# icbi-lab/infercnvpy

Measured on AMD Instinct MI355X. Metric: cells/sec through tl.infercnv (window=100), input resident in HBM, higher is better.
Workload: dtype f64

## Files before the change

include/infercnv_hip.h:

```cpp
#ifndef INFERCNV_HIP_H
#define INFERCNV_HIP_H

#include <stdint.h>

#ifdef __cplusplus
extern "C" {
#endif

typedef enum {
    ICV_OK = 0,
    ICV_ERR_INVALID = 1,
    ICV_ERR_UNSUPPORTED = 2,
    ICV_ERR_HIP = 3,
    ICV_ERR_NOMEM = 4
} icv_status;

enum { ICV_F32 = 0, ICV_F64 = 1 };
enum { ICV_DENSE = 0, ICV_CSR = 1 };

enum {
    ICV_FLAG_TRUNC_TO_INT = 1,
    ICV_FLAG_ROUND_F32 = 2,
    ICV_FLAG_NO_APPLY = 4
};
// ... 8 lines not shown
    const void *values;
    const int64_t *indptr;
    const int32_t *indices;
    int64_t csr_begin;
    int64_t csr_end;
} icv_matrix;

typedef struct icv_plan_s *icv_plan_t;

typedef struct {
    int32_t n_cols_all;
    int32_t n_genes_used;
    int32_t n_chr;
    int32_t window;
    int32_t step;
    int32_t n_windows;
    int32_t block;
    int32_t n_blocks;
    int32_t padded_len;
    int32_t lds_bytes_f32;
    int32_t lds_bytes_f64;
    int32_t workgroups_per_cu_f32;
} icv_plan_info;

int icv_plan_create(int32_t n_cols_all, const int32_t *h_col_pos, int32_t n_chr,
                    const int32_t *h_chrom_offsets, int32_t window, int32_t step, icv_plan_t *out);
void icv_plan_destroy(icv_plan_t plan);
int icv_plan_get_info(icv_plan_t plan, icv_plan_info *h_info);
int icv_plan_chr_pos(icv_plan_t plan, int32_t *h_chr_pos );
int icv_plan_window_table(icv_plan_t plan, int32_t *h_start , int32_t *h_len );
enum {
    ICV_KERNEL_NONE = 0,
    ICV_KERNEL_GENERIC = 1,
    ICV_KERNEL_WS = 2,
    ICV_KERNEL_WS_CSR = 3,
    ICV_KERNEL_X16 = 4,
    ICV_KERNEL_SD = 5,
    ICV_KERNEL_SPLIT = 6
};
int icv_plan_last_kernel(icv_plan_t plan, int32_t *h_kind);
int icv_plan_se_tables(icv_plan_t plan, int32_t *h_applies, int32_t *h_col_block ,
                       int32_t *h_col_offset , int32_t *h_block_gene0 ,
                       uint32_t *h_w0 , uint32_t *h_w1 );
int icv_plan_gene_runs(icv_plan_t plan, int32_t *h_n_runs, int32_t *h_run_first, int32_t *h_run_count,
                       int32_t *h_run_genes, int32_t *h_col_run );

int icv_colsum(const icv_matrix *m, const int32_t *row_group, int32_t n_groups, double *sums,
               void *stream);

int icv_colchain(const icv_matrix *m, const int32_t *rows, int64_t n_sel, double scale, void *acc, void *stream);
int icv_colsum_pairwise(const void *xt, int32_t dtype, int64_t n_rows, int32_t n_cols, int64_t ld, void *sums,
                        void *stream);
int icv_colchain_mean(const void *acc, int32_t dtype, int32_t n_cols, int64_t count, void *mean, void *stream);
int icv_colmean_csc(const void *values, int32_t dtype, const int64_t *colptr, const int32_t *row_idx, int32_t n_cols,
                    const int32_t *row_group, int32_t group, double scale, void *mean, void *stream);

int icv_infercnv_smooth(icv_plan_t plan, const icv_matrix *m, const void *ref_lo, const void *ref_hi,
                        double lfc_clip, int32_t flags, float *out, int64_t ldo, double *cell_median,
                        double *cell_stats, void *stream);

int icv_chunk_thresholds(const double *cell_stats, int64_t n_rows, int64_t chunksize, int64_t row_phase,
                         int32_t n_windows, double dynamic_threshold, double *thr, void *stream);

int icv_apply_threshold(icv_plan_t plan, const icv_matrix *m, const void *ref_lo, const void *ref_hi,
                        double lfc_clip, int32_t flags, float *out, int64_t ldo,
                        const double *cell_median, const double *thr, int64_t chunksize,
                        int64_t row_phase, void *stream);

typedef struct {
    float smooth_ms;
    float thresholds_ms;
    float apply_ms;
    float total_ms;
} icv_profile;

int icv_infercnv_run(icv_plan_t plan, const icv_matrix *m, const void *ref_lo, const void *ref_hi,
                     double lfc_clip, double dynamic_threshold, int64_t chunksize, int64_t row_phase,
                     int32_t flags, float *out, int64_t ldo, double *cell_median, double *cell_stats,
                     double *thr, icv_profile *h_profile, void *stream);

int icv_profile_begin(icv_plan_t plan);
int icv_profile_collect(icv_plan_t plan, icv_profile *out, int32_t max_records, int32_t *n_records);

int icv_colchain_blocks_workspace(int64_t n_rows, int32_t n_cols, int64_t *bytes);
int icv_colchain_blocks_sums(const icv_matrix *m, void *workspace, double *total, void *stream);
int icv_colchain_blocks_records(const icv_matrix *m, void *workspace, const double *est_start, void *stream);
int icv_colchain_blocks_scan(const icv_matrix *m, void *workspace, float *acc, int32_t col0, int32_t col1,
                             uint64_t *d_replayed, void *stream);

int icv_infercnv_run_windows(icv_plan_t plan, const icv_matrix *m, const void *ref_lo, const void *ref_hi,
                             double lfc_clip, double dynamic_threshold, int64_t chunksize, int64_t row_phase,
                             int32_t flags, float *out, int64_t ldo, double *cell_median, double *cell_stats,
                             double *thr, icv_profile *h_profile, double *win_out, int64_t ldw, void *stream);
int icv_gene_values_from_windows(icv_plan_t plan, const double *win, int64_t ldw, int64_t n_rows,
                                 const double *thr, int64_t chunksize, int64_t row_phase, double *gene_out,
                                 int64_t ldg, void *stream);
int icv_gene_values(icv_plan_t plan, const icv_matrix *m, const void *ref_lo, const void *ref_hi,
                    double lfc_clip, int32_t flags, const double *thr, int64_t chunksize,
                    int64_t row_phase, double *gene_out, int64_t ldg, void *stream);

int icv_csr_count(const float *x, int64_t n_rows, int32_t n_cols, int64_t ld, int64_t *row_nnz, void *stream);
int icv_csr_fill(const float *x, int64_t n_rows, int32_t n_cols, int64_t ld, const int64_t *indptr,
                 int32_t *indices, double *data, void *stream);

typedef struct {
    int32_t rows_per_round;
    int32_t mask_streamed;
    int32_t mask_ring_slots;
    int32_t mask_lds_bytes;
    int32_t mask_loads_in_flight;
    int32_t fill_streamed;
    int32_t fill_ring_slots;
    int32_t fill_lds_bytes;
    int32_t fill_loads_in_flight;
    int32_t fill_stage_entries;
} icv_pack_info;
int icv_pack_geometry(int32_t n_windows, icv_pack_info *h_info);

int icv_threshold_mask(icv_plan_t plan, const icv_matrix *m, const void *ref_lo, const void *ref_hi,
                       double lfc_clip, int32_t flags, const float *out, int64_t ldo, const double *cell_median,
                       const double *thr, int64_t chunksize, int64_t row_phase, uint64_t *mask,
                       int64_t *row_nnz, void *stream);
int icv_csr_fill_masked(const float *x, int64_t n_rows, int32_t n_cols, int64_t ld, const uint64_t *mask,
                        const int64_t *indptr, int32_t *indices, double *data, void *stream);
int icv_row_offsets(const int64_t *row_nnz, int64_t n_rows, int64_t *indptr, void *stream);

int icv_threshold_pack(icv_plan_t plan, const icv_matrix *m, const void *ref_lo, const void *ref_hi, double lfc_clip,
                       int32_t flags, const float *out, int64_t ldo, const double *cell_median, const double *thr,
                       int64_t chunksize, int64_t row_phase, int64_t *indptr, int32_t *indices, double *data,
                       int64_t capacity, void *stream);

int icv_corr_iqr(const float *x, int64_t n, int32_t k, int64_t ld, double *h_iqr, void *stream);

int icv_pairwise_sqeuclidean(const float *x, int64_t n, int32_t d, int64_t ld, int64_t row_begin, int64_t row_end,
                             float *out, int64_t ldo, void *stream);
int icv_ward_linkage(float *dist_sq, int64_t n, int64_t ld, int32_t spare_columns, double *h_linkage,
                     int32_t *h_rounds, void *stream);

#define ICV_SUPER_ROWS 1024
int icv_pairwise_sqeuclidean_tiles(const float *x, int64_t n, int32_t d, int64_t ld, int32_t n_tiles,
                                   const int32_t *h_row0, const int32_t *h_col0, const int64_t *h_dir_off,
                                   const int64_t *h_mir_off, float *dir, int64_t ld_dir, float *mir, int64_t ld_mir,
                                   void *stream);

typedef struct icv_ward_s *icv_ward_t;
int icv_ward_create(int64_t n, const int32_t *h_sr_local, int32_t n_super, int32_t super_shift, int64_t ld,
                    int32_t spare_columns, icv_ward_t *out, void *stream);
void icv_ward_destroy(icv_ward_t w);
int icv_ward_merge(icv_ward_t w, float *d_local, int64_t ld, const float *stage, int64_t ld_stage,
                   const int32_t *h_pslot, int32_t scatter, void *stream);
int icv_ward_gather(icv_ward_t w, const float *d_local, int64_t ld, const int64_t *d_rows, int32_t n_rows,
                    const int32_t *d_slots, int32_t n_slots, float *out, int64_t ldo, void *stream);
int icv_ward_scatter(icv_ward_t w, float *d_local, int64_t ld, const float *v, int64_t ldv, const int32_t *h_vrow_p,
                     int32_t n_v, void *stream);
int icv_ward_scan(icv_ward_t w, const float *d_local, int64_t ld, void *stream);
int icv_ward_pack_nn(icv_ward_t w, int32_t *d_nn, float *d_dmin, void *stream);
int icv_ward_unpack_nn(icv_ward_t w, const int32_t *d_nn, const float *d_dmin, void *stream);
int icv_ward_pairs(icv_ward_t w, float *d_local, int64_t ld, int32_t all_active, int32_t *h_counts ,
                   void *stream);
int icv_ward_round_pairs(icv_ward_t w, int32_t *h_i, int32_t *h_j);
int icv_ward_finish(icv_ward_t w, double *h_linkage, int32_t *h_rounds);

int icv_row_abs_sum(const float *x, int64_t n_rows, int32_t n_cols, int64_t ld, double *row_sum,
                    void *stream);

int icv_csr_row_abs_sum(const void *data, int32_t dtype, const int64_t *indptr, int64_t n_rows, double *row_sum,
                        void *stream);

int icv_group_sums(const double *values, const int32_t *group, int64_t n, int32_t n_groups, double *sums,
                   int64_t *counts, void *stream);

int icv_csr_check(const int64_t *indptr, const int32_t *indices, int64_t n_rows, int32_t n_cols, int64_t capacity,
                  void *stream);
int icv_csr_densify(const void *data, int32_t dtype, const int64_t *indptr, const int32_t *indices, const int64_t *rows,
                    int64_t n_sel, int32_t n_cols, float *out, int64_t ldo, void *stream);

#define ICV_GRAM_BLOCK 8192
int icv_gram_f64(const icv_matrix *m, int32_t panel_dtype, void *panel, int64_t panel_ld, double *g, int64_t ldg,
// ... 47 lines not shown
```

infercnvpy_amd/_engine.py:

```python
from __future__ import annotations

import ctypes as C
import math
import os
import time as _time

import numpy as np
import scipy.sparse as sp

from . import _lib
from ._plan import GenePlan


def _torch():
    import torch

    if not torch.cuda.is_available():
        raise RuntimeError("infercnvpy_amd needs an AMD GPU (torch.cuda.is_available() is False); "
                           "there is no CPU fallback")
    return torch


def _stream_ptr(torch):
    return C.c_void_p(torch.cuda.current_stream().cuda_stream)
# ... 161 lines not shown
        if not count:
            raise ValueError("column_chain: CSR input needs the row count of the group")
        scale = 1.0 / float(count)
    _lib.check(lib.icv_colchain(C.byref(m), _ptr(rows_d), n_sel, scale, C.c_void_p(acc_ptr), _stream_ptr(torch)))
    return acc


class ChainBlocks:

    def __init__(self, dm: "DeviceMatrix", row0=0, row1=None):
        torch = _torch()
        lib = _lib.load()
        self.dm = dm
        self.m = dm.c_struct(row0, row1)
        nbytes = C.c_int64(0)
        _lib.check(lib.icv_colchain_blocks_workspace(self.m.n_rows, self.m.n_cols, C.byref(nbytes)))
        self.ws = torch.empty(int(nbytes.value), dtype=torch.uint8, device="cuda")
        self.replayed = torch.zeros(1, dtype=torch.int64, device="cuda")

    def sums(self):
        torch = _torch()
        total = torch.empty(self.m.n_cols, dtype=torch.float64, device="cuda")
        _lib.check(_lib.load().icv_colchain_blocks_sums(C.byref(self.m), _ptr(self.ws), _ptr(total), _stream_ptr(torch)))
        return total

    def records(self, est_start=None):
        torch = _torch()
        if est_start is not None:
            assert est_start.dtype == torch.float64 and est_start.is_cuda and est_start.numel() == self.m.n_cols
            est_start = est_start.contiguous()
        _lib.check(_lib.load().icv_colchain_blocks_records(C.byref(self.m), _ptr(self.ws), _ptr(est_start),
                                                           _stream_ptr(torch)))

    def scan(self, acc, cols=None):
        torch = _torch()
        assert acc.dtype == torch.float32 and acc.is_cuda and acc.numel() == self.m.n_cols and acc.is_contiguous()
        c0, c1 = (0, self.m.n_cols) if cols is None else (int(cols[0]), int(cols[1]))
        _lib.check(_lib.load().icv_colchain_blocks_scan(C.byref(self.m), _ptr(self.ws), _ptr(acc), c0, c1,
                                                        _ptr(self.replayed), _stream_ptr(torch)))
        return acc

    def n_blocks(self):
        return (-(-int(self.m.n_rows) // 64)) * int(self.m.n_cols)


def chain_mean(acc, count, is_csr):
    if is_csr:
        return acc
    torch = _torch()
    lib = _lib.load()
    out = torch.empty_like(acc)
    _lib.check(lib.icv_colchain_mean(_ptr(acc), _lib.ICV_F32 if acc.dtype == torch.float32 else _lib.ICV_F64,
                                     acc.numel(), int(count), _ptr(out), _stream_ptr(torch)))
    return out


def csc_column_means(X, row_group=None, n_groups=1, counts=None, np_dtype=None, max_entries=1 << 28):
    torch = _torch()
    lib = _lib.load()
    X = X.tocsc()
    if not X.has_canonical_format:
        X = X.copy()
        X.sum_duplicates()
    np_dtype = np.dtype(np_dtype or (np.float32 if X.dtype == np.float32 else np.float64))
    tdt = torch.float32 if np_dtype == np.float32 else torch.float64
    code = _lib.ICV_F32 if np_dtype == np.float32 else _lib.ICV_F64
    n_cols = X.shape[1]
    indptr = X.indptr.astype(np.int64, copy=False)
    out = np.zeros((n_groups, n_cols), dtype=np_dtype)
    rg = None
    if row_group is not None:
        rg = torch.from_numpy(np.ascontiguousarray(row_group, dtype=np.int32)).cuda()
    if counts is None:
        counts = [X.shape[0]] * n_groups
    c = 0
    while c < n_cols:
        c1 = int(np.searchsorted(indptr, indptr[c] + max_entries, side="right")) - 1
        c1 = min(n_cols, max(c1, c + 1))
        e0, e1 = int(indptr[c]), int(indptr[c1])
        vals = torch.from_numpy(np.ascontiguousarray(X.data[e0:e1].astype(np_dtype, copy=False))).cuda()
        rows = torch.from_numpy(np.ascontiguousarray(X.indices[e0:e1].astype(np.int32, copy=False))).cuda()
        ptr = torch.from_numpy(np.ascontiguousarray(indptr[c:c1 + 1] - e0)).cuda()
        if e1 == e0:
            vals = torch.zeros(1, dtype=tdt, device="cuda")
            rows = torch.zeros(1, dtype=torch.int32, device="cuda")
        for g in range(n_groups):
            mean = torch.empty(c1 - c, dtype=tdt, device="cuda")
            _lib.check(lib.icv_colmean_csc(_ptr(vals), code, _ptr(ptr), _ptr(rows), c1 - c, _ptr(rg), g,
                                           1.0 / float(counts[g]), _ptr(mean), _stream_ptr(torch)))
            out[g, c:c1] = mean.cpu().numpy()
        c = c1
    return out


def fortran_column_means(X, np_dtype=None, max_bytes=1 << 30):
    torch = _torch()
    lib = _lib.load()
    n, g = X.shape
    np_dtype = np.dtype(np_dtype or (np.float32 if X.dtype == np.float32 else np.float64))
    tdt = torch.float32 if np_dtype == np.float32 else torch.float64
    code = _lib.ICV_F32 if np_dtype == np.float32 else _lib.ICV_F64
    XT = X.T
    out = np.empty(g, dtype=np_dtype)
    per = int(max(1, max_bytes // max(1, n * np_dtype.itemsize)))
    for c0 in range(0, g, per):
        c1 = min(g, c0 + per)
# ... 294 lines not shown
            th.start()

    @property
    def h2d_seconds(self):
        return max(self._busy)

    def pieces(self):
        torch = _torch()
        for k in range(len(self.bounds)):
            if k >= self._landed:
                for q in self._queues:
                    ev = q.get()
                    if ev is None:
                        raise self._err
                    torch.cuda.current_stream().wait_event(ev)
                self._landed += 1
            yield self.bounds[k]
        self._join()

    def _join(self):
        for th in self._threads:
            if th.is_alive():
                th.join()

    def close(self, cancel=False):
        if cancel:
            self._cancel.set()
        self._join()
        bufs_q = getattr(self, "_pack_bufs", None)
        if bufs_q is not None:
            self._pack_bufs = None
            while True:
                try:
                    _pack_pool_give(bufs_q.get_nowait())
                except Exception:
                    break
        if self.dm is not None:
            torch = _torch()
            cur = torch.cuda.current_stream()
            for t in self.dm._keep:
                t.record_stream(cur)
                for st in self._streams:
                    t.record_stream(st)
        self.dm = None


class PackedRows:

    def __init__(self, out, mask, counts, thr):
        self.out, self.mask, self.counts, self.thr = out, mask, counts, thr


def threshold_mask(plan: GenePlan, dm: DeviceMatrix, ref_lo, ref_hi, res, *, lfc_clip, chunksize, row_phase=0,
                   flags=0, row0=0, row1=None):
    torch = _torch()
    lib = _lib.load()
    rows = res.out.shape[0]
    n_words = (plan.n_windows + 63) // 64
    mask = torch.empty((rows, n_words), dtype=torch.int64, device="cuda")
    counts = torch.empty(rows, dtype=torch.int64, device="cuda")
    m = dm.c_struct(row0, row1)
    _lib.check(lib.icv_threshold_mask(
        plan.handle, C.byref(m), _ptr(ref_lo), _ptr(ref_hi), float(lfc_clip), int(flags), _ptr(res.out),
        res.out.stride(0), _ptr(res.cell_median), _ptr(res.thr), int(chunksize), int(row_phase), _ptr(mask),
        _ptr(counts), _stream_ptr(torch)))
    return PackedRows(res.out, mask, counts, res.thr)


class PackedCsr:

    def __init__(self, indptr, indices, data, n_cols, thr=None):
        self.indptr, self.indices, self.data, self.n_cols, self.thr = indptr, indices, data, n_cols, thr

    @property
    def n_rows(self):
        return self.indptr.shape[0] - 1

    @property
    def shape(self):
        return (self.n_rows, self.n_cols)

    @property
    def device(self):
        return self.indptr.device

    def nnz(self):
        return int(self.indptr[-1].item())

    def to_scipy(self):
        ip = self.indptr.cpu().numpy()
        n = int(ip[-1])
        return sp.csr_matrix((self.data[:n].cpu().numpy(), self.indices[:n].cpu().numpy(), ip),
                             shape=(self.n_rows, self.n_cols))

    def toarray(self):
        return self.to_scipy().toarray()

    def dense_rows(self, rows=None):
        torch = _torch()
        lib = _lib.load()
        with torch.cuda.device(self.device):
            rows_d, n_sel = None, self.n_rows
            if rows is not None:
                rows = np.asarray(rows)
                if rows.dtype == bool:
                    if rows.shape[0] != self.n_rows:
                        raise IndexError("boolean row mask of the wrong length")
                    rows = np.flatnonzero(rows)
                rows = np.ascontiguousarray(rows, dtype=np.int64)
                if rows.size and (rows.min() < 0 or rows.max() >= self.n_rows):
                    raise IndexError("row index out of range")
                n_sel = int(rows.shape[0])
                rows_d = torch.from_numpy(rows).cuda()
            ld = (self.n_cols + 3) // 4 * 4
            out = torch.empty((n_sel, max(ld, 1)), dtype=torch.float32, device="cuda")[:, :self.n_cols]
            code = _lib.ICV_F32 if self.data.dtype == torch.float32 else _lib.ICV_F64
            _lib.check(lib.icv_csr_densify(_ptr(self.data), code, _ptr(self.indptr), _ptr(self.indices), _ptr(rows_d),
                                           n_sel, self.n_cols, _ptr(out), out.stride(0), _stream_ptr(torch)))
        return out


def threshold_csr(plan: GenePlan, dm: DeviceMatrix, ref_lo, ref_hi, res, *, lfc_clip, chunksize, row_phase=0,
                  flags=0, row0=0, row1=None, capacity=None, single_pass=False):
    torch = _torch()
    lib = _lib.load()
    rows = res.out.shape[0]
    W = plan.n_windows
    if (dm.shape[0] if row1 is None else row1) - row0 == 0:
        return PackedCsr(torch.zeros(1, dtype=torch.int64, device="cuda"), torch.empty(1, dtype=torch.int32, device="cuda"),
                         torch.empty(1, dtype=torch.float64, device="cuda"), W, res.thr)
    if single_pass and W <= 20480:
        return threshold_pack(plan, dm, ref_lo, ref_hi, res, lfc_clip=lfc_clip, chunksize=chunksize,
                              row_phase=row_phase, flags=flags, row0=row0, row1=row1, capacity=capacity)
    part = threshold_mask(plan, dm, ref_lo, ref_hi, res, lfc_clip=lfc_clip, chunksize=chunksize, row_phase=row_phase,
                          flags=flags, row0=row0, row1=row1)
    cap = rows * W if capacity is None else max(int(capacity), rows * W)
    indptr = torch.empty(rows + 1, dtype=torch.int64, device="cuda")
    indices = torch.empty(max(cap, 1), dtype=torch.int32, device="cuda")
    data = torch.empty(max(cap, 1), dtype=torch.float64, device="cuda")
    st = _stream_ptr(torch)
    _lib.check(lib.icv_row_offsets(_ptr(part.counts), rows, _ptr(indptr), st))
    if rows:
        _lib.check(lib.icv_csr_fill_masked(_ptr(part.out), rows, W, part.out.stride(0), _ptr(part.mask), _ptr(indptr),
                                           _ptr(indices), _ptr(data), st))
    return PackedCsr(indptr, indices, data, W, res.thr)


def threshold_pack(plan: GenePlan, dm: DeviceMatrix, ref_lo, ref_hi, res, *, lfc_clip, chunksize, row_phase=0,
                   flags=0, row0=0, row1=None, capacity=None):
    torch = _torch()
    lib = _lib.load()
    rows = res.out.shape[0]
    W = plan.n_windows
    cap = rows * W if capacity is None else int(capacity)
    indptr = torch.empty(rows + 1, dtype=torch.int64, device="cuda")
    indices = torch.empty(max(cap, 1), dtype=torch.int32, device="cuda")
    data = torch.empty(max(cap, 1), dtype=torch.float64, device="cuda")
    m = dm.c_struct(row0, row1)
    _lib.check(lib.icv_threshold_pack(
        plan.handle, C.byref(m), _ptr(ref_lo), _ptr(ref_hi), float(lfc_clip), int(flags), _ptr(res.out),
        res.out.stride(0), _ptr(res.cell_median), _ptr(res.thr), int(chunksize), int(row_phase), _ptr(indptr),
        _ptr(indices), _ptr(data), cap, _stream_ptr(torch)))
    return PackedCsr(indptr, indices, data, W, res.thr)


def fill_from_mask(part, n_cols):
    torch = _torch()
    lib = _lib.load()
    n = part.counts.shape[0]
    ip = torch.zeros(n + 1, dtype=torch.int64, device="cuda")
    torch.cumsum(part.counts, 0, out=ip[1:])
    nnz = int(ip[-1].item())
    idx = torch.empty(max(nnz, 1), dtype=torch.int32, device="cuda")
    dat = torch.empty(max(nnz, 1), dtype=torch.float64, device="cuda")
    if nnz:
        _lib.check(lib.icv_csr_fill_masked(_ptr(part.out), n, n_cols, part.out.stride(0), _ptr(part.mask), _ptr(ip),
                                           _ptr(idx), _ptr(dat), _stream_ptr(torch)))
    return PackedCsr(ip, idx, dat, n_cols, part.thr)


def concat_packed(parts):
    torch = _torch()
    ips, idx, dat, thr, off = [parts[0].indptr[:1]], [], [], [], 0
    for p in parts:
        n = p.nnz()
        ips.append(p.indptr[1:] + off)
        idx.append(p.indices[:n])
        dat.append(p.data[:n])
        if p.thr is not None:
            thr.append(p.thr)
        off += n
    return PackedCsr(torch.cat(ips), torch.cat(idx), torch.cat(dat), parts[0].n_cols, torch.cat(thr) if thr else None)


# ... 692 lines not shown
```

infercnvpy_amd/_lib.py:

```python
from __future__ import annotations

import ctypes as C
import os

_HERE = os.path.dirname(os.path.abspath(__file__))
LIB_PATH = os.environ.get("INFERCNV_HIP_LIB") or os.path.join(_HERE, "libinfercnv_hip.so")

ICV_OK, ICV_ERR_INVALID, ICV_ERR_UNSUPPORTED, ICV_ERR_HIP, ICV_ERR_NOMEM = range(5)
ICV_F32, ICV_F64 = 0, 1
ICV_DENSE, ICV_CSR = 0, 1
ICV_FLAG_TRUNC_TO_INT = 1
ICV_FLAG_ROUND_F32 = 2
ICV_FLAG_NO_APPLY = 4
ICV_GRAM_BLOCK = 8192
(ICV_KERNEL_NONE, ICV_KERNEL_GENERIC, ICV_KERNEL_WS, ICV_KERNEL_WS_CSR, ICV_KERNEL_X16, ICV_KERNEL_SD,
 ICV_KERNEL_SPLIT) = range(7)

EXPORTS = (
    "icv_plan_create", "icv_plan_destroy", "icv_plan_get_info", "icv_plan_chr_pos", "icv_plan_window_table",
    "icv_plan_last_kernel", "icv_plan_se_tables", "icv_plan_gene_runs",
    "icv_colsum", "icv_colchain", "icv_colsum_pairwise", "icv_colchain_mean", "icv_colmean_csc", "icv_infercnv_smooth", "icv_chunk_thresholds", "icv_apply_threshold", "icv_infercnv_run",
    "icv_infercnv_run_windows", "icv_gene_values_from_windows",
    "icv_colchain_blocks_workspace", "icv_colchain_blocks_sums", "icv_colchain_blocks_records", "icv_colchain_blocks_scan",
    "icv_profile_begin", "icv_profile_collect",
    "icv_gene_values", "icv_csr_count", "icv_csr_fill", "icv_threshold_mask", "icv_csr_fill_masked", "icv_row_offsets", "icv_pack_geometry", "icv_threshold_pack", "icv_corr_iqr",
    "icv_pairwise_sqeuclidean", "icv_ward_linkage", "icv_pairwise_sqeuclidean_tiles",
    "icv_ward_create", "icv_ward_destroy", "icv_ward_merge", "icv_ward_gather", "icv_ward_scatter", "icv_ward_scan", "icv_ward_pack_nn",
    "icv_ward_unpack_nn", "icv_ward_pairs", "icv_ward_round_pairs", "icv_ward_finish", "icv_row_abs_sum", "icv_csr_row_abs_sum", "icv_group_sums", "icv_csr_check", "icv_csr_densify", "icv_gram_f64", "icv_project", "icv_host_dense_row_nnz", "icv_host_dense_pack", "icv_host_dense_pack_fused", "icv_csr_scatter_dense", "icv_last_error", "icv_version",
    "icv_device_count", "icv_developer_knobs_reload",
    "icv_knn_workspace", "icv_knn", "icv_knn_fuzzy", "icv_knn_symmetrize_count", "icv_knn_symmetrize_fill",
    "icv_knn_sort_rows",
    "icv_leiden_workspace", "icv_leiden_quantise", "icv_leiden_iteration", "icv_leiden_sums", "icv_leiden_renumber",
)


class Matrix(C.Structure):
    _fields_ = [
        ("format", C.c_int32), ("dtype", C.c_int32), ("n_rows", C.c_int64), ("n_cols", C.c_int32),
        ("_pad", C.c_int32), ("ld", C.c_int64), ("values", C.c_void_p), ("indptr", C.c_void_p),
        ("indices", C.c_void_p), ("csr_begin", C.c_int64), ("csr_end", C.c_int64),
    ]


class PlanInfo(C.Structure):
    _fields_ = [(n, C.c_int32) for n in (
        "n_cols_all", "n_genes_used", "n_chr", "window", "step", "n_windows", "block", "n_blocks", "padded_len",
        "lds_bytes_f32", "lds_bytes_f64", "workgroups_per_cu_f32")]


class PackInfo(C.Structure):
    _fields_ = [(n, C.c_int32) for n in (
        "rows_per_round", "mask_streamed", "mask_ring_slots", "mask_lds_bytes", "mask_loads_in_flight", "fill_streamed",
        "fill_ring_slots", "fill_lds_bytes", "fill_loads_in_flight", "fill_stage_entries")]


class Profile(C.Structure):
    _fields_ = [("smooth_ms", C.c_float), ("thresholds_ms", C.c_float), ("apply_ms", C.c_float),
                ("total_ms", C.c_float)]


class HipExtensionMissing(RuntimeError):
    pass


_lib = None


def load():
    global _lib
    if _lib is not None:
        return _lib
    if not os.path.exists(LIB_PATH):
        raise HipExtensionMissing(
            f"{LIB_PATH} not found: build it with `python -m infercnvpy_amd._build` "
            "(hipcc --offload-arch=gfx950).  infercnvpy_amd has no CPU fallback."
        )
    import torch

    lib = C.CDLL(LIB_PATH)
    i32, i64, vp, dbl = C.c_int32, C.c_int64, C.c_void_p, C.c_double
    P = C.POINTER
    lib.icv_plan_create.argtypes = [i32, vp, i32, vp, i32, i32, P(vp)]
    lib.icv_plan_destroy.argtypes = [vp]
    lib.icv_plan_destroy.restype = None
    lib.icv_plan_get_info.argtypes = [vp, P(PlanInfo)]
    lib.icv_plan_chr_pos.argtypes = [vp, vp]
    lib.icv_plan_window_table.argtypes = [vp, vp, vp]
    lib.icv_plan_last_kernel.argtypes = [vp, P(i32)]
    lib.icv_plan_se_tables.argtypes = [vp, P(i32), vp, vp, vp, vp, vp]
    lib.icv_plan_gene_runs.argtypes = [vp, P(i32), vp, vp, vp, vp]
    lib.icv_colsum.argtypes = [P(Matrix), vp, i32, vp, vp]
    lib.icv_colchain.argtypes = [P(Matrix), vp, i64, dbl, vp, vp]
    lib.icv_colsum_pairwise.argtypes = [vp, i32, i64, i32, i64, vp, vp]
    lib.icv_colchain_mean.argtypes = [vp, i32, i32, i64, vp, vp]
    lib.icv_colmean_csc.argtypes = [vp, i32, vp, vp, i32, vp, i32, dbl, vp, vp]
    lib.icv_infercnv_smooth.argtypes = [vp, P(Matrix), vp, vp, dbl, i32, vp, i64, vp, vp, vp]
    lib.icv_chunk_thresholds.argtypes = [vp, i64, i64, i64, i32, dbl, vp, vp]
    lib.icv_apply_threshold.argtypes = [vp, P(Matrix), vp, vp, dbl, i32, vp, i64, vp, vp, i64, i64, vp]
    lib.icv_infercnv_run.argtypes = [vp, P(Matrix), vp, vp, dbl, dbl, i64, i64, i32, vp, i64, vp, vp, vp,
                                     P(Profile), vp]
    lib.icv_infercnv_run_windows.argtypes = [vp, P(Matrix), vp, vp, dbl, dbl, i64, i64, i32, vp, i64, vp, vp, vp,
                                             P(Profile), vp, i64, vp]
    lib.icv_gene_values_from_windows.argtypes = [vp, vp, i64, i64, vp, i64, i64, vp, i64, vp]
    lib.icv_colchain_blocks_workspace.argtypes = [i64, i32, P(i64)]
    lib.icv_colchain_blocks_sums.argtypes = [P(Matrix), vp, vp, vp]
    lib.icv_colchain_blocks_records.argtypes = [P(Matrix), vp, vp, vp]
    lib.icv_colchain_blocks_scan.argtypes = [P(Matrix), vp, vp, i32, i32, vp, vp]
    lib.icv_profile_begin.argtypes = [vp]
    lib.icv_profile_collect.argtypes = [vp, P(Profile), i32, P(i32)]
    lib.icv_gene_values.argtypes = [vp, P(Matrix), vp, vp, dbl, i32, vp, i64, i64, vp, i64, vp]
    lib.icv_csr_count.argtypes = [vp, i64, i32, i64, vp, vp]
    lib.icv_csr_fill.argtypes = [vp, i64, i32, i64, vp, vp, vp, vp]
    lib.icv_threshold_mask.argtypes = [vp, P(Matrix), vp, vp, dbl, i32, vp, i64, vp, vp, i64, i64, vp, vp, vp]
    lib.icv_threshold_pack.argtypes = [vp, P(Matrix), vp, vp, dbl, i32, vp, i64, vp, vp, i64, i64, vp, vp, vp, i64, vp]
    lib.icv_row_offsets.argtypes = [vp, i64, vp, vp]
    lib.icv_pack_geometry.argtypes = [i32, P(PackInfo)]
    lib.icv_csr_fill_masked.argtypes = [vp, i64, i32, i64, vp, vp, vp, vp, vp]
    lib.icv_corr_iqr.argtypes = [vp, i64, i32, i64, P(C.c_double), vp]
    lib.icv_pairwise_sqeuclidean.argtypes = [vp, i64, i32, i64, i64, i64, vp, i64, vp]
    lib.icv_ward_linkage.argtypes = [vp, i64, i64, i32, vp, P(i32), vp]
    lib.icv_pairwise_sqeuclidean_tiles.argtypes = [vp, i64, i32, i64, i32, vp, vp, vp, vp, vp, i64, vp, i64, vp]
    lib.icv_ward_create.argtypes = [i64, vp, i32, i32, i64, i32, P(vp), vp]
    lib.icv_ward_destroy.argtypes = [vp]
    lib.icv_ward_destroy.restype = None
    lib.icv_ward_merge.argtypes = [vp, vp, i64, vp, i64, vp, i32, vp]
    lib.icv_ward_gather.argtypes = [vp, vp, i64, vp, i32, vp, i32, vp, i64, vp]
    lib.icv_ward_scatter.argtypes = [vp, vp, i64, vp, i64, vp, i32, vp]
    lib.icv_ward_scan.argtypes = [vp, vp, i64, vp]
    lib.icv_ward_pack_nn.argtypes = [vp, vp, vp, vp]
    lib.icv_ward_unpack_nn.argtypes = [vp, vp, vp, vp]
    lib.icv_ward_pairs.argtypes = [vp, vp, i64, i32, P(i32), vp]
    lib.icv_ward_round_pairs.argtypes = [vp, vp, vp]
    lib.icv_ward_finish.argtypes = [vp, vp, P(i32)]
    lib.icv_row_abs_sum.argtypes = [vp, i64, i32, i64, vp, vp]
    lib.icv_csr_row_abs_sum.argtypes = [vp, i32, vp, i64, vp, vp]
    lib.icv_group_sums.argtypes = [vp, vp, i64, i32, vp, vp, vp]
    lib.icv_csr_check.argtypes = [vp, vp, i64, i32, i64, vp]
    lib.icv_csr_densify.argtypes = [vp, i32, vp, vp, vp, i64, i32, vp, i64, vp]
    lib.icv_gram_f64.argtypes = [P(Matrix), i32, vp, i64, vp, i64, i32, vp]
    lib.icv_project.argtypes = [P(Matrix), vp, i32, vp, i32, vp, i64, vp]
    lib.icv_host_dense_row_nnz.argtypes = [vp, i32, i64, i64, i64, vp, i32]
    lib.icv_host_dense_pack.argtypes = [vp, i32, i64, i64, i64, vp, vp, vp, i32]
    lib.icv_host_dense_pack_fused.argtypes = [vp, i32, i64, i64, i64, vp, vp, vp, i64, i32, vp]
    lib.icv_csr_scatter_dense.argtypes = [vp, i32, vp, vp, i64, i32, vp, i64, vp]
    lib.icv_knn_workspace.argtypes = [i64, i32, i32, P(i64)]
    lib.icv_knn.argtypes = [vp, i64, i32, i64, i32, vp, vp, vp, P(i32), P(C.c_float), vp]
    lib.icv_knn_fuzzy.argtypes = [vp, i64, i32, vp, vp, vp, vp]
    lib.icv_knn_symmetrize_count.argtypes = [vp, vp, i64, i32, vp, vp]
    lib.icv_knn_symmetrize_fill.argtypes = [vp, vp, i64, i32, vp, i64, vp, vp, vp]
    lib.icv_knn_sort_rows.argtypes = [vp, i64, vp, vp, vp, vp, vp]
    lib.icv_leiden_workspace.argtypes = [i64, i64, P(i64)]
    lib.icv_leiden_quantise.argtypes = [vp, vp, vp, i32, i64, i64, i32, vp, vp, vp, P(i64), vp]
    lib.icv_leiden_iteration.argtypes = [vp, vp, vp, i64, i64, dbl, C.c_uint64, i32, vp, vp, P(i32), P(i32), P(i64),
                                         P(i32), P(C.c_float), vp]
    lib.icv_leiden_sums.argtypes = [vp, vp, vp, i64, vp, vp, vp, vp]
    lib.icv_leiden_renumber.argtypes = [vp, i64, vp, P(i32), vp]
    lib.icv_developer_knobs_reload.restype = None
    lib.icv_developer_knobs_reload.argtypes = []
    lib.icv_last_error.restype = C.c_char_p
    lib.icv_last_error.argtypes = []
    for name in EXPORTS:
        fn = getattr(lib, name)
        if name not in ("icv_plan_destroy", "icv_ward_destroy", "icv_last_error", "icv_developer_knobs_reload"):
            fn.restype = C.c_int
    _lib = lib
    return lib


# ... 16 lines not shown
```

infercnvpy_amd/csrc/icv_api.hip:

```cpp
#include "../../include/infercnv_hip.h"

#include <hip/hip_runtime.h>

#include <algorithm>
#include <atomic>
#include <cmath>
#include <cstdio>
#include <cstdlib>
#include <cstring>
#include <mutex>
#include <new>
#include <string>
#include <system_error>
#include <thread>
#if defined(__x86_64__)
#include <immintrin.h>
#endif
#include <memory>
#include <vector>

#include <rocprim/device/device_radix_sort.hpp>
#include <rocprim/device/device_reduce_by_key.hpp>
#include <rocprim/device/device_scan.hpp>

// ... 44 lines not shown
        no_x16 = std::getenv("ICV_NO_X16") != nullptr;
        no_sd = std::getenv("ICV_NO_SD") != nullptr;
        phase_profile = std::getenv("ICV_PHASE_PROFILE") != nullptr;
        ward_in_place = std::getenv("ICV_WARD_IN_PLACE") != nullptr;
        no_mask_ring = std::getenv("ICV_NO_MASK_RING") != nullptr;
        no_fill_ring = std::getenv("ICV_NO_FILL_RING") != nullptr;
        no_chain_queues = std::getenv("ICV_NO_CHAIN_QUEUES") != nullptr;
        se_maxw4 = std::getenv("ICV_SE_MAXW4") != nullptr;
        no_gene_fused = std::getenv("ICV_NO_GENE_FUSED") != nullptr;
        const char* e = std::getenv("ICV_WGS_PER_CU");
        wgs_per_cu = e ? std::atoi(e) : 0;
        e = std::getenv("ICV_CHAIN_FAR");
        chain_far = e ? std::atoi(e) : 0;
        e = std::getenv("ICV_CHAIN_PIECES");
        chain_pieces = e ? std::atoi(e) : 0;
        e = std::getenv("ICV_WARD_COMPACT_X");
        ward_compact_x = e ? std::atof(e) : 0.0;
    }
};
std::mutex g_knobs_mu;
bool g_knobs_loaded = false;
Knobs g_knobs;
const Knobs& knobs() {
    std::lock_guard<std::mutex> lk(g_knobs_mu);
    if (!g_knobs_loaded) {
        g_knobs.load();
        g_knobs_loaded = true;
    }
    return g_knobs;
}

}

struct icv_plan_s {
    icv::Plan p;
    std::mutex mu;
    std::atomic<bool> busy{false};
    int device = -1;
    int n_cu = 0;
    int32_t *d_dst = nullptr, *d_src = nullptr, *d_wstart = nullptr, *d_wlen = nullptr;
    double* d_wdenom = nullptr;
    int32_t* d_pad = nullptr;
    int32_t* d_wpack = nullptr;
    unsigned* d_tie_n = nullptr;
    int32_t *d_cov_col = nullptr, *d_cov_j0 = nullptr, *d_cov_cnt = nullptr;
    uint32_t* d_gv_pk = nullptr;
    int32_t* d_gv_mult = nullptr;
    uint16_t* d_gv_col16 = nullptr;
    bool gv_fused_ok = false;
    int gv_mult_bytes = 2;
    int64_t* d_row_list = nullptr;
    int* d_row_count = nullptr;
    int64_t row_list_cap = 0;
    bool prof_deferred = false;
    std::vector<hipEvent_t> prof_events;
    double* d_win_scratch = nullptr;
    int64_t win_scratch_cap = 0;
    double* d_cell_part = nullptr;
    int64_t cell_part_cap = 0;
    double* d_chunk_part = nullptr;
    int64_t chunk_part_cap = 0;
    double* d_hb_stats = nullptr;
    int64_t hb_stats_cap = 0;
    uint16_t* d_dst16 = nullptr;
    uint32_t* d_x16_wdesc = nullptr;
    int32_t* d_blk_g0 = nullptr;
    uint32_t *d_se_w0 = nullptr, *d_se_w1 = nullptr;
    void* d_zrow = nullptr;
    size_t zrow_elems = 0;
    std::vector<icv_plan_s*> parts;
    std::vector<int> part_woff;
    int parts_elem = 0;
    int last_kernel = ICV_KERNEL_NONE;
    hipEvent_t done_ev = nullptr;
    hipStream_t last_stream = nullptr;
    bool has_last = false;
};

namespace {

int64_t se_grid(const icv_plan_t pl, int64_t n_rows) {
    int per_cu = icv::kLdsLimit / icv::kSeLds;
    if (const int v = knobs().wgs_per_cu)
        if (v >= 1 && v < per_cu) per_cu = v;
    int64_t grid = (int64_t)pl->n_cu * per_cu;
    return grid > n_rows ? n_rows : grid;
}

struct PlanBusy {
    icv_plan_t pl;
    bool ok;
    hipStream_t st = nullptr;
    bool entered = false;
    explicit PlanBusy(icv_plan_t p) : pl(p), ok(false) {
        bool expected = false;
        ok = p && p->busy.compare_exchange_strong(expected, true);
    }
    hipError_t enter(hipStream_t s) {
        st = s;
        entered = true;
        if (!pl->done_ev) {
            const hipError_t e = hipEventCreateWithFlags(&pl->done_ev, hipEventDisableTiming);
            if (e != hipSuccess) return e;
        }
        if (pl->has_last && pl->last_stream != s) return hipStreamWaitEvent(s, pl->done_ev, 0);
        return hipSuccess;
// ... 23 lines not shown
    hipError_t alloc(size_t bytes, hipStream_t s) {
        st = s;
        keep_pool();
        return hipMallocAsync(&p, bytes ? bytes : 16, s);
    }
    static void keep_pool() {
        static std::atomic<unsigned long long> done{0};
        int dev = 0;
        if (hipGetDevice(&dev) != hipSuccess || dev < 0 || dev > 63) return;
        const unsigned long long bit = 1ull << dev;
        if (done.fetch_or(bit) & bit) return;
        hipMemPool_t pool;
        if (hipDeviceGetDefaultMemPool(&pool, dev) == hipSuccess) {
            uint64_t keep = 6ull << 30;
            (void)hipMemPoolSetAttribute(pool, hipMemPoolAttrReleaseThreshold, &keep);
        }
    }
    template <typename T>
    T* as() const { return static_cast<T*>(p); }
};
struct EventSet {
    hipEvent_t ev[4] = {nullptr, nullptr, nullptr, nullptr};
    bool keep = false;
    ~EventSet() {
        if (!keep)
            for (auto& e : ev)
                if (e) (void)hipEventDestroy(e);
    }
};

int ensure_device(icv_plan_t pl) {
    std::lock_guard<std::mutex> lk(pl->mu);
    int dev = 0;
    HIP_TRY(hipGetDevice(&dev));
    if (pl->device == dev) return ICV_OK;
    if (pl->device >= 0) return fail(ICV_ERR_INVALID, "plan is bound to another device");
    const icv::Plan& p = pl->p;
    hipDeviceProp_t prop;
    HIP_TRY(hipGetDeviceProperties(&prop, dev));
    pl->n_cu = prop.multiProcessorCount;
    auto up = [&](const void* h, size_t bytes, void** d) -> hipError_t {
        hipError_t e = hipMalloc(d, bytes ? bytes : 16);
        if (e != hipSuccess) return e;
        return bytes ? hipMemcpy(*d, h, bytes, hipMemcpyHostToDevice) : hipSuccess;
    };
    HIP_TRY(up(p.dst.data(), p.dst.size() * 4 + 0, (void**)&pl->d_dst));
    HIP_TRY(up(p.src.data(), p.src.size() * 4, (void**)&pl->d_src));
    HIP_TRY(up(p.w_start.data(), p.w_start.size() * 4, (void**)&pl->d_wstart));
    HIP_TRY(up(p.w_len.data(), p.w_len.size() * 4, (void**)&pl->d_wlen));
    HIP_TRY(up(p.w_denom.data(), p.w_denom.size() * 8, (void**)&pl->d_wdenom));
    HIP_TRY(up(p.pad_idx.data(), p.pad_idx.size() * 4, (void**)&pl->d_pad));
    HIP_TRY(up(p.w_pack.data(), p.w_pack.size() * 4, (void**)&pl->d_wpack));
    {
        const unsigned zeros[2] = {0u, 0u};
        HIP_TRY(up(zeros, sizeof(zeros), (void**)&pl->d_tie_n));
    }
    HIP_TRY(up(p.cov_col.data(), p.cov_col.size() * 4, (void**)&pl->d_cov_col));
    HIP_TRY(up(p.cov_j0.data(), p.cov_j0.size() * 4, (void**)&pl->d_cov_j0));
    HIP_TRY(up(p.cov_cnt.data(), p.cov_cnt.size() * 4, (void**)&pl->d_cov_cnt));
    {
        const size_t R = p.gv_run_j0.size();
        bool ok = p.W <= 65535 && R < 65535;
        std::vector<uint32_t> pk(R);
        for (size_t r = 0; r < R && ok; ++r) {
            ok = p.gv_run_cnt[r] <= 128 && p.gv_run_mult[r] <= 65535;
            pk[r] = (uint32_t)p.gv_run_j0[r] | ((uint32_t)p.gv_run_cnt[r] << 16);
        }
        std::vector<uint16_t> c16(((size_t)p.n_cols_all + 7) / 8 * 8, (uint16_t)R);
        for (int c = 0; c < p.n_cols_all && ok; ++c) c16[c] = p.gv_col_run[c] < 0 ? (uint16_t)R : (uint16_t)p.gv_col_run[c];
        pl->gv_fused_ok = ok;
        pl->gv_mult_bytes = 1;
        for (int32_t v : p.gv_run_mult)
            if (v > 255) pl->gv_mult_bytes = 2;
        HIP_TRY(up(pk.data(), pk.size() * 4, (void**)&pl->d_gv_pk));
        HIP_TRY(up(p.gv_run_mult.data(), p.gv_run_mult.size() * 4, (void**)&pl->d_gv_mult));
        HIP_TRY(up(c16.data(), c16.size() * 2, (void**)&pl->d_gv_col16));
    }
    HIP_TRY(up(p.dst16.data(), p.dst16.size() * 2, (void**)&pl->d_dst16));
    HIP_TRY(up(p.x16_wdesc.data(), p.x16_wdesc.size() * 4, (void**)&pl->d_x16_wdesc));
    HIP_TRY(up(p.blk_g0.data(), p.blk_g0.size() * 4, (void**)&pl->d_blk_g0));
    HIP_TRY(up(p.se_w0.data(), p.se_w0.size() * 4, (void**)&pl->d_se_w0));
    HIP_TRY(up(p.se_w1.data(), p.se_w1.size() * 4, (void**)&pl->d_se_w1));
    pl->zrow_elems = (size_t)icv::round_up(p.Gp, 4) + 4;
    HIP_TRY(hipMalloc(&pl->d_zrow, pl->zrow_elems * 8));
    pl->device = dev;
    return ICV_OK;
}

int check_matrix(const icv_plan_t pl, const icv_matrix* m) {
    if (!pl || !m) return fail(ICV_ERR_INVALID, "null plan or matrix");
    if (m->n_cols != pl->p.n_cols_all)
        return fail(ICV_ERR_INVALID, "matrix has " + std::to_string(m->n_cols) + " columns, plan expects " +
                                         std::to_string(pl->p.n_cols_all));
    if (m->dtype != ICV_F32 && m->dtype != ICV_F64) return fail(ICV_ERR_INVALID, "dtype must be ICV_F32 or ICV_F64");
    if (m->format != ICV_DENSE && m->format != ICV_CSR) return fail(ICV_ERR_INVALID, "format must be dense or csr");
    if (m->n_rows < 0) return fail(ICV_ERR_INVALID, "negative n_rows");
    if (m->n_rows > 0 && !m->values && !(m->format == ICV_CSR)) return fail(ICV_ERR_INVALID, "null values");
    if (m->format == ICV_DENSE && m->ld < m->n_cols) return fail(ICV_ERR_INVALID, "ld < n_cols");
    if (m->format == ICV_CSR && (!m->indptr || (!m->indices && m->values)))
        return fail(ICV_ERR_INVALID, "csr needs indptr and indices");
    return ICV_OK;
}

bool aligned16(const void* p) { return (reinterpret_cast<uintptr_t>(p) & 15u) == 0; }

int build_parts(icv_plan_t pl, int elem_bytes) {
    std::lock_guard<std::mutex> lk(pl->mu);
    if (pl->parts_elem >= elem_bytes) return ICV_OK;
// ... 119 lines not shown
        HIP_TRY(hipMemset(d, 0, 32 * sizeof(unsigned long long)));
        icv::KParams K2 = K;
        K2.dbg = d;
        hipLaunchKernelGGL(kern, dim3((unsigned)grid), dim3(block), lds, st, K2);
        HIP_TRY(hipStreamSynchronize(st));
        unsigned long long h[32];
        HIP_TRY(hipMemcpy(h, d, sizeof(h), hipMemcpyDeviceToHost));
        if (block == icv::XT) {
            (void)hipFree(d);
            std::fprintf(stderr, "[icv x16 profile] grid=%lld rows=%lld lds=%d cycles per cell: A: store %.0f, chains %.0f, S "
                                 "%.0f, barrier 1 %.0f, B: output+gather+clear %.0f, W %.0f, L %.0f, barrier 2 %.0f\n", (long long)grid,
                         (long long)K.n_rows, lds, (double)h[6] / (double)K.n_rows, (double)h[7] / (double)K.n_rows,
                         (double)h[0] / (double)K.n_rows, (double)h[1] / (double)K.n_rows,
                         (double)h[4] / (double)K.n_rows, (double)h[5] / (double)K.n_rows,
                         (double)h[2] / (double)K.n_rows, (double)h[3] / (double)K.n_rows);
            return ICV_OK;
        }
        (void)hipFree(d);
        if (lds == icv::kSeLds) {
            std::fprintf(stderr, "[icv se profile] grid=%lld rows=%lld cycles per cell of the profiled thread:", (long long)grid,
                         (long long)K.n_rows);
            const char* nm[8] = {"ph0", "A", "ph1", "B1", "ph2", "B2", "ph3", "B3"};
            for (int i = 0; i < 8; ++i) std::fprintf(stderr, " %s %.0f", nm[i], (double)h[i] / (double)K.n_rows);
            std::fprintf(stderr, "\n");
            return ICV_OK;
        }
        const char* names[6] = {"L load+scatter", "S block sums", "W windows", "M2 rank/select", "O output",
                                "M1 pivot search"};
        double tot = 0;
        for (int i = 0; i < 6; ++i) tot += (double)h[i];
        std::fprintf(stderr, "[icv phase profile] grid=%lld rows=%lld lds=%d\n", (long long)grid,
                     (long long)K.n_rows, lds);
        for (int i = 0; i < 6; ++i)
            std::fprintf(stderr, "  %-16s %12.0f cycles/cell  %5.1f %%\n", names[i], (double)h[i] / (double)K.n_rows,
                         100.0 * (double)h[i] / tot);
        std::fprintf(stderr, "  [6] %.2f  [7] %.4f per cell (fast: median iterations, split cells; ws: phases are "
                             "A-wait, gather+L, B1-wait, S+emit, S01+B3, W+B4; [6] = selector scan cycles, [7] = fallback cells)\n",
                     (double)h[6] / (double)K.n_rows, (double)h[7] / (double)K.n_rows);
        return ICV_OK;
    }
    hipLaunchKernelGGL(kern, dim3((unsigned)grid), dim3(block), lds, st, K);
    HIP_TRY(hipGetLastError());
    return ICV_OK;
}

bool x16_applies(const icv_plan_t pl, const icv_matrix* m, const icv::KParams& K, const icv::Layout& lay) {
    const icv::Plan& p = pl->p;
    return lay.fits && m->dtype == ICV_F32 && m->format == ICV_DENSE && p.ws_ok && K.vec_ok && std::isfinite(K.cap) &&
           !knobs().force_generic && p.x16_ok && !K.bounded && !knobs().no_x16 &&
           p.step == 10 &&
           ((p.B == 10 && p.window == 100 && p.x16_fine == 4096) || (p.B == 5 && p.window == 250 && p.x16_fine == 1024));
}

int hand_back_workspace(icv_plan_t pl, icv::KParams& K, hipStream_t st) {
    if (pl->row_list_cap < K.n_rows) {
        (void)hipFree(pl->d_row_list);
        pl->d_row_list = nullptr;
        pl->row_list_cap = 0;
        HIP_TRY(hipMalloc((void**)&pl->d_row_list, (size_t)K.n_rows * sizeof(int64_t)));
        pl->row_list_cap = K.n_rows;
    }
    if (pl->cell_part_cap < K.n_rows) {
        (void)hipFree(pl->d_cell_part);
        pl->d_cell_part = nullptr;
        pl->cell_part_cap = 0;
        HIP_TRY(hipMalloc((void**)&pl->d_cell_part, (size_t)K.n_rows * 32 * sizeof(double)));
        pl->cell_part_cap = K.n_rows;
    }
    K.cell_part = pl->d_cell_part;
    if (!pl->d_row_count) HIP_TRY(hipMalloc((void**)&pl->d_row_count, sizeof(int)));
    HIP_TRY(hipMemsetAsync(pl->d_row_count, 0, sizeof(int), st));
    K.row_list = pl->d_row_list;
    K.row_count = pl->d_row_count;
    return ICV_OK;
}

int launch_hand_back(icv_plan_t pl, const icv::KParams& K, hipStream_t st, bool csr) {
    const icv::Plan& p = pl->p;
    icv::KParams G = K;
    G.win_off = p.lay32.win_off;
    G.scratch_off = p.lay32.scratch_off;
    G.dbg = nullptr;
    const int need = (p.NB + icv::kThreads - 1) / icv::kThreads;
    void (*gk)(const icv::KParams);
    if (csr) gk = need <= 4 ? icv::k_smooth<float, true, 4> : icv::k_smooth<float, true, 8>;
    else gk = need <= 4 ? icv::k_smooth<float, false, 4> : icv::k_smooth<float, false, 8>;
    HIP_TRY(hipFuncSetAttribute(reinterpret_cast<const void*>(gk), hipFuncAttributeMaxDynamicSharedMemorySize,
                                p.lay32.total));
    int64_t g2 = pl->n_cu;
    if (g2 > K.n_rows) g2 = K.n_rows;
    hipLaunchKernelGGL(gk, dim3((unsigned)g2), dim3(icv::NT), p.lay32.total, st, G);
    HIP_TRY(hipGetLastError());
    return ICV_OK;
}

bool se_fraction_bits(const icv::Plan& p, double cap, int* k0, int* k1) {
    if (!p.se_ok || knobs().no_sd) return false;
    int e = 0;
    (void)std::frexp((double)p.B * 2.0 * cap + 1.0, &e);
    const int a = 51 - e;
    (void)std::frexp((double)p.B * (double)(p.B - 1) * cap + 1.0, &e);
    const int b = 51 - e;
    if (a < 40 || b < 36) return false;
    *k0 = a;
    *k1 = b;
    return true;
}

bool stored_entries_kernel(const icv_plan_t pl, const icv_matrix* m, const icv::KParams& K, const icv::Layout& lay) {
    if (!(lay.fits && m->dtype == ICV_F32 && m->format == ICV_CSR && std::isfinite(K.cap) &&
          m->csr_end > m->csr_begin && !knobs().force_generic))
        return false;
    int k0 = 0, k1 = 0;
    return se_fraction_bits(pl->p, K.cap, &k0, &k1);
}

int launch_smooth_se(icv_plan_t pl, icv::KParams K, hipStream_t st, hipEvent_t kernel_done = nullptr,
                     int64_t csr_entries = 0, int row_len_hint = 0) {
    const icv::Plan& p = pl->p;
    int k0 = 0, k1 = 0;
    if (!se_fraction_bits(p, K.cap, &k0, &k1)) return fail(ICV_ERR_INVALID, "k_smooth_se does not apply");
    AsyncBuf tab_guard, hi_guard, wt_guard, g_guard;
    const int nz = (int)pl->zrow_elems;
    hipLaunchKernelGGL(icv::k_zero_row<float>, dim3((nz + 255) / 256), dim3(256), 0, st, K,
                       static_cast<float*>(pl->d_zrow), nz);
    HIP_TRY(tab_guard.alloc((size_t)K.n_cols * 16, st));
    HIP_TRY(wt_guard.alloc((size_t)p.W * 16, st));
    HIP_TRY(g_guard.alloc((size_t)(p.NB + 8) * 8, st));
    if (K.bounded) HIP_TRY(hi_guard.alloc((size_t)K.n_cols * 4, st));
    K.sd_tab = tab_guard.p;
    K.sd_tab_hi = K.bounded ? hi_guard.as<float>() : nullptr;
    K.sd_wtab = wt_guard.p;
    K.sd_g16 = g_guard.as<double>();
    K.sd_scale = std::ldexp(1.0, k0);
    K.sd_qinv = std::ldexp(1.0, -k0);
    K.sd_q1inv = std::ldexp(1.0, -k1);
    K.sd_r = std::ldexp(1.0, k1 - k0);
    K.sd_window = p.window;
    hipLaunchKernelGGL(icv::k_se_table, dim3((unsigned)((K.n_cols + 255) / 256)), dim3(256), 0, st, K,
                       tab_guard.as<icv::u32x4>(), const_cast<float*>(K.sd_tab_hi), (float)std::ldexp(1.0, k1));
    const int n_wt = p.W > p.NB + 8 ? p.W : p.NB + 8;
    hipLaunchKernelGGL(icv::k_se_wtab, dim3((unsigned)((n_wt + 255) / 256)), dim3(256), 0, st, K,
                       static_cast<const float*>(pl->d_zrow), pl->d_se_w0, pl->d_se_w1, wt_guard.as<icv::u32x4>(),
                       g_guard.as<double>(), K.sd_r);
    if (int rc = hand_back_workspace(pl, K, st)) return rc;
    int64_t grid = se_grid(pl, K.n_rows);
    if (grid < 1) {
        if (kernel_done) HIP_TRY(hipEventRecord(kernel_done, st));
        return ICV_OK;
    }
    void (*kern)(const icv::KParams);
    const bool w3 = p.W <= 3 * icv::NT && !knobs().se_maxw4;
    int pf = 4;
    if (K.chunk_part && !knobs().se_maxw4 && K.n_rows > 0) {
        double want = 0.0;
        if (row_len_hint > 0) {
            want = (double)row_len_hint;
        } else if (csr_entries > 0) {
            const double mean = (double)csr_entries / (double)K.n_rows;
            const double dens = mean / (double)(K.n_cols > 0 ? K.n_cols : 1);
            want = mean + 3.5 * std::sqrt(mean * (dens < 1.0 ? 1.0 - dens : 0.0)) + 8.0;
        }
        if (want > 0.0) pf = want <= icv::NT ? 1 : want <= 2 * icv::NT ? 2 : want <= 3 * icv::NT ? 3 : 4;
    }
#define ICV_SE_PICK(MW, CH, BD)                                                                              \
    (pf == 1 ? icv::k_smooth_se<MW, CH, BD, 1> : pf == 2 ? icv::k_smooth_se<MW, CH, BD, 2>                   \
     : pf == 3 ? icv::k_smooth_se<MW, CH, BD, 3> : icv::k_smooth_se<MW, CH, BD, 4>)
    if (K.win_out) {
        if (!K.chunk_part) return fail(ICV_ERR_INVALID, "k_smooth_se with windows needs the chunk-moment mode");
        if (w3) kern = K.bounded ? icv::k_smooth_se<3, true, true, 4, true> : icv::k_smooth_se<3, true, false, 4, true>;
        else kern = K.bounded ? icv::k_smooth_se<4, true, true, 4, true> : icv::k_smooth_se<4, true, false, 4, true>;
    } else if (K.chunk_part) {
        if (w3) kern = K.bounded ? ICV_SE_PICK(3, true, true) : ICV_SE_PICK(3, true, false);
        else kern = K.bounded ? ICV_SE_PICK(4, true, true) : ICV_SE_PICK(4, true, false);
    } else {
        if (w3) kern = K.bounded ? icv::k_smooth_se<3, false, true> : icv::k_smooth_se<3, false, false>;
        else kern = K.bounded ? icv::k_smooth_se<4, false, true> : icv::k_smooth_se<4, false, false>;
    }
#undef ICV_SE_PICK
    int rc = run_kernel(kern, grid, icv::kSeLds, K, st);
    if (kernel_done && !rc) HIP_TRY(hipEventRecord(kernel_done, st));
    if (rc) return rc;
    if (!K.chunk_part)
        hipLaunchKernelGGL(icv::k_stats_finish, dim3((unsigned)((K.n_rows + 255) / 256)), dim3(256), 0, st, K.cell_part,
                           K.n_rows, K.cell_stats);
    pl->last_kernel = ICV_KERNEL_SD;
    return launch_hand_back(pl, K, st, true);
}

int launch_smooth_fast(icv_plan_t pl, icv::KParams K, hipStream_t st, bool csr, int64_t csr_begin, int64_t csr_end,
                       hipEvent_t kernel_done = nullptr) {
    const icv::Plan& p = pl->p;
    const int need_b = (p.NB + icv::kThreads - 1) / icv::kThreads;
    void (*kern)(const icv::KParams) = nullptr;
    constexpr int U = icv::kFastUMax;
    K.scratch_off = p.fast_scratch_off;
    AsyncBuf ws_guard;
    void* ws_buf = nullptr;
    const int lds = p.fast_lds;
    if (!p.ws_ok) return -1;
    {
        const bool u10 = (p.B == 10 && p.window == 100);
        if (!csr) {
            if (need_b <= 4) kern = u10 ? icv::k_smooth_ws<U, 4, 4, 10, 10, false> : icv::k_smooth_ws<U, 4, 4, 0, 0, false>;
            else if (p.B == 5 && p.window == 250) kern = icv::k_smooth_ws<U, 8, 4, 5, 50, false>;
            else kern = (p.B == 5) ? icv::k_smooth_ws<U, 8, 4, 5, 0, false> : icv::k_smooth_ws<U, 8, 4, 0, 0, false>;
        } else {
            const int nz = (int)pl->zrow_elems;
            hipLaunchKernelGGL(icv::k_zero_row<float>, dim3((nz + 255) / 256), dim3(256), 0, st, K,
                               static_cast<float*>(pl->d_zrow), nz);
            const int64_t n = csr_end - csr_begin;
            int64_t g = (n + 255) / 256;
            if (g > 8192) g = 8192;
            if (need_b <= 4) kern = u10 ? icv::k_smooth_ws<U, 4, 4, 10, 10, true> : icv::k_smooth_ws<U, 4, 4, 0, 0, true>;
            else kern = (p.B == 5) ? icv::k_smooth_ws<U, 8, 4, 5, 0, true> : icv::k_smooth_ws<U, 8, 4, 0, 0, true>;
            HIP_TRY(ws_guard.alloc((size_t)(n > 0 ? n : 1) * 6, st));
            ws_buf = ws_guard.p;
            float* cv = static_cast<float*>(ws_buf);
            uint16_t* ps = reinterpret_cast<uint16_t*>(cv + (n > 0 ? n : 1));
            K.cvals = cv - csr_begin;
            K.pos16 = ps - csr_begin;
            if (n > 0)
                hipLaunchKernelGGL(icv::k_csr_prepare, dim3((unsigned)g), dim3(256), 0, st, K, csr_begin, csr_end,
                                   const_cast<uint16_t*>(K.pos16), const_cast<float*>(K.cvals));
        }
        K.hist_off = p.ws_hist_off;
        if (int rc = hand_back_workspace(pl, K, st)) return rc;
    }
    int per_cu = icv::kLdsLimit / lds;
    if (per_cu > 4) per_cu = 4;
    if (const int v = knobs().wgs_per_cu)
        if (v >= 1 && v < per_cu) per_cu = v;
    int64_t grid = (int64_t)pl->n_cu * per_cu;
    if (grid > K.n_rows) grid = K.n_rows;
    if (grid < 1) {
        if (kernel_done) HIP_TRY(hipEventRecord(kernel_done, st));
        return ICV_OK;
    }
    int rc;
    void (*xk)(const icv::KParams) = nullptr;
    if (!csr && p.x16_ok && !K.bounded && !knobs().no_x16) {
        if (p.step != 10)
            xk = nullptr;
        else if (p.B == 10 && p.window == 100 && p.x16_fine == 4096)
            xk = K.win_out ? icv::k_smooth_x16<10, 10, 1, true, 4096, true, true>
                           : (K.chunk_part ? icv::k_smooth_x16<10, 10, 1, true, 4096, true>
                                           : icv::k_smooth_x16<10, 10, 1, false, 4096, true>);
        else if (p.B == 5 && p.window == 250 && p.x16_fine == 1024)
            xk = K.win_out ? icv::k_smooth_x16<5, 50, 2, true, 1024, false, true>
                           : (K.chunk_part ? icv::k_smooth_x16<5, 50, 2, true, 1024, false>
                                           : icv::k_smooth_x16<5, 50, 2, false, 1024, false>);
    }
    if (K.win_out && (!xk || !K.chunk_part)) return -1;
    if (xk) {
        icv::KParams X = K;
        X.win_off = p.x16_s01_off;
        X.hist_off = p.x16_hist_off;
        X.scratch_off = p.x16_scratch_off;
        int64_t gx = pl->n_cu;
        if (gx > K.n_rows) gx = K.n_rows;
        rc = run_kernel(xk, gx, p.x16_lds, X, st, icv::XT);
        if (kernel_done && !rc) HIP_TRY(hipEventRecord(kernel_done, st));
        if (rc) return rc;
        if (!K.chunk_part)
            hipLaunchKernelGGL(icv::k_stats_finish_n, dim3((unsigned)((K.n_rows + 255) / 256)), dim3(256), 0, st,
                               K.cell_part, K.n_rows, icv::XWAVE, K.cell_stats);
    } else {
        rc = run_kernel(kern, grid, lds, K, st);
        if (kernel_done && !rc) HIP_TRY(hipEventRecord(kernel_done, st));
        if (rc) return rc;
        hipLaunchKernelGGL(icv::k_stats_finish, dim3((unsigned)((K.n_rows + 255) / 256)), dim3(256), 0, st,
                           K.cell_part, K.n_rows, K.cell_stats);
    }
    pl->last_kernel = xk ? ICV_KERNEL_X16 : (csr ? ICV_KERNEL_WS_CSR : ICV_KERNEL_WS);
    return launch_hand_back(pl, K, st, csr);
}

template <typename T, bool CSR>
int launch_smooth_t(icv_plan_t pl, const icv::KParams& K, const icv::Layout& lay, hipStream_t st) {
    const icv::Plan& p = pl->p;
// ... 131 lines not shown
                                      : launch_smooth_t<float, true>(pl, K, lay, st);
    return m->format == ICV_DENSE ? launch_smooth_t<double, false>(pl, K, lay, st)
                                  : launch_smooth_t<double, true>(pl, K, lay, st);
}

int launch_apply(const icv_matrix* m, const icv::KParams& K, const double* thr, int64_t chunksize,
                 int64_t row_phase, hipStream_t st) {
    if (K.n_rows < 1) return ICV_OK;
    dim3 grid((unsigned)K.n_rows), block(256);
    if (m->dtype == ICV_F32) {
        if (m->format == ICV_DENSE)
            hipLaunchKernelGGL((icv::k_apply_thr<float, false>), grid, block, 0, st, K, thr, chunksize, row_phase);
        else
            hipLaunchKernelGGL((icv::k_apply_thr<float, true>), grid, block, 0, st, K, thr, chunksize, row_phase);
    } else {
        if (m->format == ICV_DENSE)
            hipLaunchKernelGGL((icv::k_apply_thr<double, false>), grid, block, 0, st, K, thr, chunksize, row_phase);
        else
            hipLaunchKernelGGL((icv::k_apply_thr<double, true>), grid, block, 0, st, K, thr, chunksize, row_phase);
    }
    HIP_TRY(hipGetLastError());
    return ICV_OK;
}

}

namespace {
int current_cu_count() {
    static std::atomic<int> cached[64];
    int dev = 0;
    if (hipGetDevice(&dev) != hipSuccess || dev < 0 || dev > 63) return 256;
    int n = cached[dev].load(std::memory_order_relaxed);
    if (n > 0) return n;
    hipDeviceProp_t prop;
    n = hipGetDeviceProperties(&prop, dev) == hipSuccess ? prop.multiProcessorCount : 256;
    cached[dev].store(n, std::memory_order_relaxed);
    return n;
}

__global__ void k_chain_line_tiles(int n_lines, int grid, uint16_t* line_tile) {
    const int t = blockIdx.x * blockDim.x + threadIdx.x;
    if (t >= grid) return;
    const int l0 = (int)((int64_t)t * n_lines / grid), l1 = (int)((int64_t)(t + 1) * n_lines / grid);
    for (int l = l0; l < l1; ++l) line_tile[l] = (uint16_t)t;
}

template <typename T>
__global__ void k_chain_mean(const T* acc, int n, T denom, T* out) {
    const int i = blockIdx.x * blockDim.x + threadIdx.x;
    if (i < n) out[i] = acc[i] / denom;
}

template <typename T>
int colchain_dense(const icv_matrix* m, const int32_t* rows, int64_t n_sel, T* acc, hipStream_t st) {
    const icv::ChainLaunch L(m->n_cols, (int)sizeof(T), current_cu_count());
    constexpr int EPL = 16 / (int)sizeof(T);
    int64_t tail = -1, n_dma = n_sel;
    if ((int64_t)(m->_pad > 0 ? m->_pad : 0) + (int64_t)(m->n_cols + EPL - 1) / EPL * EPL > m->ld) {
        tail = m->n_rows - 1;
        if (!rows) n_dma = n_sel - 1;
    }
    typedef void (*kern_t)(const T*, int64_t, int, int, int, const int32_t*, int64_t, int64_t, T*);
    const kern_t kern = rows ? (kern_t)icv::k_colchain<T, true> : (kern_t)icv::k_colchain<T, false>;
    HIP_TRY(hipFuncSetAttribute(reinterpret_cast<const void*>(kern), hipFuncAttributeMaxDynamicSharedMemorySize,
                                icv::kChLdsFull));
    hipLaunchKernelGGL(kern, dim3(L.dense_grid), dim3(icv::kChThreads), L.lds_bytes, st, (const T*)m->values, m->ld,
                       m->n_cols, L.n_units, L.lds_bytes, rows, n_dma, tail, acc);
    HIP_TRY(hipGetLastError());
    return ICV_OK;
}

template <typename T>
int colchain_csr(const icv_matrix* m, const int32_t* rows, int64_t n_sel, double scale, T* acc, hipStream_t st) {
    const icv::ChainLaunch L(m->n_cols, (int)sizeof(T), current_cu_count());
    if (L.grid > 65535) return fail(ICV_ERR_UNSUPPORTED, "icv_colchain: more than 65535 column tiles");
    AsyncBuf lt_b, bounds_b;
    HIP_TRY(lt_b.alloc((size_t)L.n_lines * sizeof(uint16_t), st));
    const int esz_shift_q = sizeof(T) == 4 ? 2 : 3;
    const size_t tab_lds = (size_t)icv::kQTabRows * (size_t)((L.grid + 2) | 1) * sizeof(uint16_t) +
                           (size_t)L.n_lines * sizeof(uint16_t);
    if (m->n_cols <= 65535 && tab_lds <= 160 * 1024 && !knobs().no_chain_queues) {
        hipLaunchKernelGGL(k_chain_line_tiles, dim3((L.grid + 255) / 256), dim3(256), 0, st, L.n_lines, L.grid,
                           lt_b.as<uint16_t>());
        const int64_t n_tb = (n_sel + icv::kQTabRows - 1) / icv::kQTabRows;
        HIP_TRY(bounds_b.alloc((size_t)n_tb * (L.grid + 1) * icv::kQTabRows * sizeof(uint16_t), st));
        typedef void (*tb_t)(const int64_t*, const int32_t*, const int32_t*, int64_t, const uint16_t*, int, int, int,
                             uint32_t*);
        const tb_t tb = rows ? (tb_t)icv::k_csr_tile_bounds16<true> : (tb_t)icv::k_csr_tile_bounds16<false>;
        if (tab_lds > 48 * 1024)
            HIP_TRY(hipFuncSetAttribute(reinterpret_cast<const void*>(tb), hipFuncAttributeMaxDynamicSharedMemorySize,
                                        (int)tab_lds));
        hipLaunchKernelGGL(tb, dim3((unsigned)n_tb), dim3(256), tab_lds, st, m->indptr, m->indices, rows, n_sel,
                           lt_b.as<uint16_t>(), L.n_lines, esz_shift_q, L.grid, bounds_b.as<uint32_t>());
        typedef void (*kq_t)(const T*, const int64_t*, const int32_t*, int64_t, const int32_t*, int64_t, int, int, int,
                             const uint16_t*, T, int, T*);
        int pieces = 4;
        {
            const double rows_all = m->n_rows > 0 ? (double)m->n_rows : 1.0;
            double per_row = (double)(m->csr_end - m->csr_begin) / rows_all;
            if (m->_pad > 0 && (double)m->_pad > per_row) per_row = (double)m->_pad;
            const int tile_lines = (L.n_lines + L.grid - 1) / L.grid;
            const double mu = per_row * (double)(tile_lines * (128 / (int)sizeof(T))) / (double)(m->n_cols > 0 ? m->n_cols : 1);
            pieces = mu <= 2.0 ? 2 : mu <= 8.5 ? 4 : mu <= 28.0 ? 8 : 16;
            const int forced = knobs().chain_pieces;
            if (forced == 2 || forced == 4 || forced == 8 || forced == 16) pieces = forced;
        }
#define ICV_KQ(P) (rows ? (kq_t)icv::k_colchain_csrq<T, true, P> : (kq_t)icv::k_colchain_csrq<T, false, P>)
        const kq_t kq = pieces == 2 ? ICV_KQ(2) : pieces == 4 ? ICV_KQ(4) : pieces == 8 ? ICV_KQ(8) : ICV_KQ(16);
#undef ICV_KQ
        HIP_TRY(hipFuncSetAttribute(reinterpret_cast<const void*>(kq), hipFuncAttributeMaxDynamicSharedMemorySize,
                                    icv::kChLdsFull));
        hipLaunchKernelGGL(kq, dim3(L.grid), dim3(icv::kChThreads), icv::kChLdsFull, st, (const T*)m->values, m->indptr,
                           m->indices, m->n_rows, rows, n_sel, m->n_cols, L.n_lines, icv::kChLdsFull,
                           (const uint16_t*)bounds_b.as<uint16_t>(), (T)scale,
                           knobs().chain_far > 0 ? knobs().chain_far : icv::kQFar, acc);
        HIP_TRY(hipGetLastError());
        return ICV_OK;
    }
    const int64_t n_blk = (n_sel + icv::kCcBlock - 1) / icv::kCcBlock;
    HIP_TRY(bounds_b.alloc((size_t)n_blk * (L.grid + 1) * icv::kCcBlock * sizeof(uint32_t), st));
// ... 286 lines not shown
    const BlocksLayout L(m->n_rows, m->n_cols);
    char* w = static_cast<char*>(workspace);
    const double* partial = reinterpret_cast<const double*>(w + L.partial_off);
    double* slab_start = reinterpret_cast<double*>(w + L.start_off);
    HIP_TRY(hipMemsetAsync(w + L.count_off, 0, 256, st));
    hipLaunchKernelGGL(icv::k_blocks_prefix, dim3((m->n_cols + 255) / 256), dim3(256), 0, st, partial, (int)L.n_slabs,
                       m->n_cols, est_start, slab_start);
    dim3 grid((m->n_cols + 255) / 256, (unsigned)L.n_slabs);
    hipLaunchKernelGGL(icv::k_chain_records, grid, dim3(256), 0, st, (const float*)m->values, m->n_rows, m->ld, m->n_cols,
                       slab_start, reinterpret_cast<uint32_t*>(w + L.rec_off), reinterpret_cast<uint32_t*>(w + L.slab_rec_off),
                       reinterpret_cast<float*>(w + L.stash_off), reinterpret_cast<unsigned*>(w + L.count_off), L.stash_cap);
    HIP_TRY(hipGetLastError());
    return ICV_OK;
}

int icv_colchain_blocks_scan(const icv_matrix* m, void* workspace, float* acc, int32_t col0, int32_t col1,
                             uint64_t* d_replayed, void* stream) {
    int rc = blocks_check(m, workspace);
    if (rc) return rc;
    if (!acc || col0 < 0 || col1 > m->n_cols || col0 > col1) return fail(ICV_ERR_INVALID, "bad colchain_blocks_scan arguments");
    if (m->n_rows == 0 || col1 == col0) return ICV_OK;
    hipStream_t st = static_cast<hipStream_t>(stream);
    const BlocksLayout L(m->n_rows, m->n_cols);
    char* w = static_cast<char*>(workspace);
    const int nc = col1 - col0;
    int64_t grid = ((int64_t)nc + 3) / 4;
    const int64_t cap = (int64_t)current_cu_count() * 8;
    if (grid > cap) grid = cap;
    hipLaunchKernelGGL(icv::k_chain_scan, dim3((unsigned)grid), dim3(256), 0, st,
                       (const float*)m->values + col0, m->n_rows, m->ld, nc, (int64_t)m->n_cols,
                       reinterpret_cast<const uint32_t*>(w + L.rec_off) + col0,
                       reinterpret_cast<const uint32_t*>(w + L.slab_rec_off) + col0,
                       reinterpret_cast<const float*>(w + L.stash_off), acc + col0,
                       reinterpret_cast<unsigned long long*>(d_replayed));
    HIP_TRY(hipGetLastError());
    return ICV_OK;
}

int icv_colchain(const icv_matrix* m, const int32_t* rows, int64_t n_sel, double scale, void* acc, void* stream) {
    if (!m || !acc) return fail(ICV_ERR_INVALID, "bad colchain arguments");
    if (m->dtype != ICV_F32 && m->dtype != ICV_F64) return fail(ICV_ERR_INVALID, "dtype must be ICV_F32 or ICV_F64");
    if (!rows) n_sel = m->n_rows;
    if (n_sel < 0 || n_sel > m->n_rows) return fail(ICV_ERR_INVALID, "icv_colchain: n_sel out of range");
    if (n_sel == 0 || m->n_cols == 0) return ICV_OK;
    hipStream_t st = static_cast<hipStream_t>(stream);
    if (m->format == ICV_CSR)
        return m->dtype == ICV_F32 ? colchain_csr<float>(m, rows, n_sel, scale, (float*)acc, st)
                                   : colchain_csr<double>(m, rows, n_sel, scale, (double*)acc, st);
    if (m->format != ICV_DENSE) return fail(ICV_ERR_INVALID, "format must be dense or csr");
    return m->dtype == ICV_F32 ? colchain_dense<float>(m, rows, n_sel, (float*)acc, st)
                               : colchain_dense<double>(m, rows, n_sel, (double*)acc, st);
}

int icv_colchain_mean(const void* acc, int32_t dtype, int32_t n_cols, int64_t count, void* mean, void* stream) {
    if (!acc || !mean || count < 1 || n_cols < 0) return fail(ICV_ERR_INVALID, "bad colchain_mean arguments");
    hipStream_t st = static_cast<hipStream_t>(stream);
    if (n_cols == 0) return ICV_OK;
    if (dtype == ICV_F32)
        hipLaunchKernelGGL(k_chain_mean<float>, dim3((n_cols + 255) / 256), dim3(256), 0, st, (const float*)acc, n_cols,
                           (float)count, (float*)mean);
    else if (dtype == ICV_F64)
        hipLaunchKernelGGL(k_chain_mean<double>, dim3((n_cols + 255) / 256), dim3(256), 0, st, (const double*)acc,
                           n_cols, (double)count, (double*)mean);
    else
        return fail(ICV_ERR_INVALID, "dtype must be ICV_F32 or ICV_F64");
    HIP_TRY(hipGetLastError());
    return ICV_OK;
}

int icv_colmean_csc(const void* values, int32_t dtype, const int64_t* colptr, const int32_t* row_idx, int32_t n_cols,
                    const int32_t* row_group, int32_t group, double scale, void* mean, void* stream) {
    if (!values || !colptr || !row_idx || !mean || n_cols < 0) return fail(ICV_ERR_INVALID, "bad colmean_csc arguments");
    hipStream_t st = static_cast<hipStream_t>(stream);
    if (n_cols == 0) return ICV_OK;
    if (dtype == ICV_F32)
        hipLaunchKernelGGL(icv::k_colpair_csc<float>, dim3((n_cols + 63) / 64), dim3(64), 0, st, (const float*)values,
                           colptr, row_idx, n_cols, row_group, group, (float)scale, (float*)mean);
    else if (dtype == ICV_F64)
        hipLaunchKernelGGL(icv::k_colpair_csc<double>, dim3((n_cols + 63) / 64), dim3(64), 0, st, (const double*)values,
                           colptr, row_idx, n_cols, row_group, group, scale, (double*)mean);
    else
        return fail(ICV_ERR_INVALID, "dtype must be ICV_F32 or ICV_F64");
    HIP_TRY(hipGetLastError());
    return ICV_OK;
}

int icv_colsum_pairwise(const void* xt, int32_t dtype, int64_t n_rows, int32_t n_cols, int64_t ld, void* sums,
                        void* stream) {
    if (!xt || !sums || n_rows < 0 || n_cols < 0 || ld < n_rows) return fail(ICV_ERR_INVALID, "bad colsum_pairwise arguments");
    hipStream_t st = static_cast<hipStream_t>(stream);
    if (n_cols == 0) return ICV_OK;
    if (dtype == ICV_F32)
        hipLaunchKernelGGL(icv::k_colpair_dense<float>, dim3((n_cols + 63) / 64), dim3(64), 0, st, (const float*)xt,
                           n_rows, n_cols, ld, (float*)sums);
    else if (dtype == ICV_F64)
        hipLaunchKernelGGL(icv::k_colpair_dense<double>, dim3((n_cols + 63) / 64), dim3(64), 0, st, (const double*)xt,
                           n_rows, n_cols, ld, (double*)sums);
    else
        return fail(ICV_ERR_INVALID, "dtype must be ICV_F32 or ICV_F64");
    HIP_TRY(hipGetLastError());
    return ICV_OK;
}

int icv_infercnv_smooth(icv_plan_t pl, const icv_matrix* m, const void* ref_lo, const void* ref_hi,
                        double lfc_clip, int32_t flags, float* out, int64_t ldo, double* cell_median,
                        double* cell_stats, void* stream) {
// ... 20 lines not shown
                       cell_stats, n_rows, chunksize, row_phase, n_windows, dynamic_threshold, thr);
    HIP_TRY(hipGetLastError());
    return ICV_OK;
}

int icv_apply_threshold(icv_plan_t pl, const icv_matrix* m, const void* ref_lo, const void* ref_hi,
                        double lfc_clip, int32_t flags, float* out, int64_t ldo, const double* cell_median,
                        const double* thr, int64_t chunksize, int64_t row_phase, void* stream) {
    int rc = check_matrix(pl, m);
    if (rc) return rc;
    PLAN_BUSY_GUARD(pl);
    if (!cell_median || !thr || chunksize < 1) return fail(ICV_ERR_INVALID, "bad apply_threshold arguments");
    if ((rc = ensure_device(pl))) return rc;
    PLAN_ENTER(stream);
    icv::KParams K;
    const icv::Layout* lay;
    if ((rc = fill_params(pl, m, ref_lo, ref_hi, lfc_clip, flags, out, ldo, const_cast<double*>(cell_median),
                          nullptr, K, lay)))
        return rc;
    return launch_apply(m, K, thr, chunksize, row_phase, static_cast<hipStream_t>(stream));
}

}

namespace {
int run_steps(icv_plan_t pl, const icv_matrix* m, const void* ref_lo, const void* ref_hi, double lfc_clip,
              double dynamic_threshold, int64_t chunksize, int64_t row_phase, int32_t flags, float* out, int64_t ldo,
              double* cell_median, double* cell_stats, double* thr, icv_profile* prof, double* win_out, int64_t ldw,
              void* stream) {
    int rc;
    const bool do_thr = !std::isnan(dynamic_threshold);
    hipStream_t st = static_cast<hipStream_t>(stream);
    icv::KParams K;
    const icv::Layout* lay;
    if ((rc = fill_params(pl, m, ref_lo, ref_hi, lfc_clip, flags, out, ldo, cell_median, cell_stats, K, lay)))
        return rc;
    K.win_out = win_out;
    K.win_ld = ldw;
    bool chunk_mode = false;
    int64_t n_chunks = 1, cs_eff = m->n_rows > 0 ? m->n_rows : 1, ph_eff = 0;
    if (do_thr) {
        cs_eff = chunksize;
        ph_eff = row_phase;
        n_chunks = (m->n_rows + row_phase + chunksize - 1) / chunksize;
        if (n_chunks < 1) n_chunks = 1;
    }
    if (!cell_stats && m->n_rows > 0) {
        if (pl->hb_stats_cap < m->n_rows) {
            (void)hipFree(pl->d_hb_stats);
            pl->d_hb_stats = nullptr;
            pl->hb_stats_cap = 0;
            HIP_TRY(hipMalloc((void**)&pl->d_hb_stats, (size_t)m->n_rows * 2 * sizeof(double)));
            pl->hb_stats_cap = m->n_rows;
        }
        K.cell_stats = pl->d_hb_stats;
        const int64_t se_slots = ((int64_t)pl->n_cu * (icv::kLdsLimit / icv::kSeLds)) * icv::NWAVE;
        const int64_t x16_slots = (int64_t)pl->n_cu * icv::XWAVE;
        const int64_t n_part = se_slots > x16_slots ? se_slots : x16_slots;
        if ((x16_applies(pl, m, K, *lay) || stored_entries_kernel(pl, m, K, *lay)) &&
            n_chunks * n_part <= (int64_t)(64 << 20) / 16) {
            chunk_mode = true;
            if (pl->chunk_part_cap < n_chunks * n_part) {
                (void)hipFree(pl->d_chunk_part);
                pl->d_chunk_part = nullptr;
                pl->chunk_part_cap = 0;
                HIP_TRY(hipMalloc((void**)&pl->d_chunk_part, (size_t)(n_chunks * n_part) * 2 * sizeof(double)));
                pl->chunk_part_cap = n_chunks * n_part;
            }
            HIP_TRY(hipMemsetAsync(pl->d_chunk_part, 0, (size_t)(n_chunks * n_part) * 2 * sizeof(double), st));
            HIP_TRY(hipMemsetAsync(pl->d_hb_stats, 0, (size_t)m->n_rows * 2 * sizeof(double), st));
            K.chunk_part = pl->d_chunk_part;
            K.chunksize = cs_eff;
            K.row_phase = ph_eff;
        }
    }
    EventSet evs;
    hipEvent_t* ev = evs.ev;
    const bool deferred = !prof && pl->prof_deferred;
    const bool timed = prof || deferred;
    if (timed) {
        for (int i = 0; i < 4; ++i) HIP_TRY(hipEventCreate(&ev[i]));
        HIP_TRY(hipEventRecord(ev[0], st));
    }
    bool ev1_done = false;
    if ((rc = launch_smooth(pl, m, K, *lay, st, timed ? ev[1] : nullptr, &ev1_done))) return rc;
    if (timed && !ev1_done) HIP_TRY(hipEventRecord(ev[1], st));
    if (do_thr && chunk_mode) {
        int64_t n_slots;
        if (m->format == ICV_CSR) {
            n_slots = se_grid(pl, m->n_rows) * icv::NWAVE;
        } else {
            int64_t gx = pl->n_cu;
            if (gx > m->n_rows) gx = m->n_rows;
            n_slots = gx * icv::XWAVE;
        }
        hipLaunchKernelGGL(icv::k_chunk_thr_part, dim3((unsigned)n_chunks), dim3(256), 0, st, pl->d_chunk_part,
                           (int)n_slots, pl->d_hb_stats, m->n_rows, chunksize, row_phase, pl->p.W,
                           dynamic_threshold, thr);
        HIP_TRY(hipGetLastError());
    } else if (do_thr && m->n_rows > 0) {
        rc = icv_chunk_thresholds(K.cell_stats, m->n_rows, chunksize, row_phase, pl->p.W, dynamic_threshold, thr,
                                  stream);
        if (rc) return rc;
    }
    if (timed) HIP_TRY(hipEventRecord(ev[2], st));
    if (do_thr && !(flags & ICV_FLAG_NO_APPLY) && (rc = launch_apply(m, K, thr, chunksize, row_phase, st))) return rc;
    if (timed) HIP_TRY(hipEventRecord(ev[3], st));
    if (deferred) {
        for (int i = 0; i < 4; ++i) pl->prof_events.push_back(ev[i]);
        evs.keep = true;
    } else if (prof) {
        HIP_TRY(hipEventSynchronize(ev[3]));
        HIP_TRY(hipEventElapsedTime(&prof->smooth_ms, ev[0], ev[1]));
        HIP_TRY(hipEventElapsedTime(&prof->thresholds_ms, ev[1], ev[2]));
        HIP_TRY(hipEventElapsedTime(&prof->apply_ms, ev[2], ev[3]));
        HIP_TRY(hipEventElapsedTime(&prof->total_ms, ev[0], ev[3]));
    }
    return ICV_OK;
}

int gene_from_windows(icv_plan_t pl, const double* win, int64_t ldw, int64_t n, const double* thr, int64_t chunksize,
                      int64_t row_phase, double* gene_out, int64_t ldg, hipStream_t st) {
    const icv::Plan& p = pl->p;
    if (n < 1) return ICV_OK;
    const int W = p.W, n_cov = (int)p.cov_col.size(), R = (int)p.gv_run_j0.size();
    const bool pk_lds = icv::gv_lds_bytes(W, R, pl->gv_mult_bytes, true) * 2 <= (size_t)icv::kLdsLimit;
    const size_t lds = icv::gv_lds_bytes(W, R, pl->gv_mult_bytes, pk_lds);
    if (lds <= (size_t)icv::kLdsLimit && pl->gv_fused_ok && !knobs().no_gene_fused) {
        HIP_TRY(hipFuncSetAttribute(reinterpret_cast<const void*>(icv::k_gene_fused),
                                    hipFuncAttributeMaxDynamicSharedMemorySize, (int)lds));
        int per_cu = (int)((size_t)icv::kLdsLimit / lds);
        if (per_cu > 2048 / icv::kGvThreads) per_cu = 2048 / icv::kGvThreads;
        int64_t grid = (int64_t)pl->n_cu * per_cu;
        if (grid > n) grid = n;
        hipLaunchKernelGGL(icv::k_gene_fused, dim3((unsigned)grid), dim3(icv::kGvThreads), lds, st, win, ldw, n, W,
                           pl->d_gv_pk, pl->d_gv_mult, R, n_cov, pl->d_gv_col16, p.n_cols_all, thr,
                           chunksize > 0 ? chunksize : 1, row_phase, gene_out, ldg, pl->gv_mult_bytes, (int)pk_lds);
        HIP_TRY(hipGetLastError());
        return ICV_OK;
    }
    AsyncBuf b_gv, b_med;
    HIP_TRY(b_gv.alloc((size_t)n * (n_cov > 0 ? n_cov : 1) * sizeof(double), st));
    HIP_TRY(b_med.alloc((size_t)n * sizeof(double), st));
    double *gv = b_gv.as<double>(), *med = b_med.as<double>();
    {
        const int64_t total = n * ldg;
        hipLaunchKernelGGL(icv::k_fill_nan, dim3((unsigned)((total + 255) / 256)), dim3(256), 0, st, gene_out, total);
    }
    if (n_cov > 0) {
        for (int64_t r0 = 0; r0 < n; r0 += 32768) {
            const int64_t nr = (n - r0) < 32768 ? (n - r0) : 32768;
            dim3 grid((n_cov + 255) / 256, (unsigned)nr);
// ... 63 lines not shown
    for (auto& e : pl->prof_events) (void)hipEventDestroy(e);
    pl->prof_events.clear();
    pl->prof_deferred = true;
    return ICV_OK;
}

int icv_profile_collect(icv_plan_t pl, icv_profile* out, int32_t max_records, int32_t* n_records) {
    if (!pl || !n_records || (max_records > 0 && !out)) return fail(ICV_ERR_INVALID, "bad profile_collect arguments");
    const int n = (int)(pl->prof_events.size() / 4);
    int k = 0;
    for (int i = 0; i < n; ++i) {
        hipEvent_t* ev = pl->prof_events.data() + 4 * i;
        if (k < max_records) {
            HIP_TRY(hipEventSynchronize(ev[3]));
            HIP_TRY(hipEventElapsedTime(&out[k].smooth_ms, ev[0], ev[1]));
            HIP_TRY(hipEventElapsedTime(&out[k].thresholds_ms, ev[1], ev[2]));
            HIP_TRY(hipEventElapsedTime(&out[k].apply_ms, ev[2], ev[3]));
            HIP_TRY(hipEventElapsedTime(&out[k].total_ms, ev[0], ev[3]));
            ++k;
        }
    }
    for (auto& e : pl->prof_events) (void)hipEventDestroy(e);
    pl->prof_events.clear();
    pl->prof_deferred = false;
    *n_records = k;
    return ICV_OK;
}

int icv_gene_values(icv_plan_t pl, const icv_matrix* m, const void* ref_lo, const void* ref_hi, double lfc_clip,
                    int32_t flags, const double* thr, int64_t chunksize, int64_t row_phase, double* gene_out,
                    int64_t ldg, void* stream) {
    int rc = check_matrix(pl, m);
    if (rc) return rc;
    PLAN_BUSY_GUARD(pl);
    if (!gene_out || ldg < m->n_cols) return fail(ICV_ERR_INVALID, "gene_out is null or ldg < n_cols");
    if (thr && (chunksize < 1 || row_phase < 0 || row_phase >= chunksize))
        return fail(ICV_ERR_INVALID, "chunksize / row_phase invalid");
    if ((rc = ensure_device(pl))) return rc;
    PLAN_ENTER(stream);
    const int64_t n = m->n_rows;
    if (n < 1) return ICV_OK;
    hipStream_t st = static_cast<hipStream_t>(stream);
    const int W = pl->p.W;
    AsyncBuf b_out32, b_win, b_cmed;
    HIP_TRY(b_out32.alloc((size_t)n * W * sizeof(float), st));
    HIP_TRY(b_win.alloc((size_t)n * W * sizeof(double), st));
    HIP_TRY(b_cmed.alloc((size_t)n * sizeof(double), st));
    if ((rc = run_steps(pl, m, ref_lo, ref_hi, lfc_clip, std::nan(""), 1, 0, flags, b_out32.as<float>(), W,
                        b_cmed.as<double>(), nullptr, nullptr, nullptr, b_win.as<double>(), W, stream)))
        return rc;
    return gene_from_windows(pl, b_win.as<double>(), W, n, thr, chunksize, row_phase, gene_out, ldg, st);
}

int icv_threshold_mask(icv_plan_t pl, const icv_matrix* m, const void* ref_lo, const void* ref_hi, double lfc_clip,
                       int32_t flags, const float* out, int64_t ldo, const double* cell_median, const double* thr,
                       int64_t chunksize, int64_t row_phase, uint64_t* mask, int64_t* row_nnz, void* stream) {
    int rc = check_matrix(pl, m);
    if (rc) return rc;
    PLAN_BUSY_GUARD(pl);
    if (!cell_median || !mask || !row_nnz || (thr && (chunksize < 1 || row_phase < 0 || row_phase >= chunksize)))
        return fail(ICV_ERR_INVALID, "bad threshold_mask arguments");
    if ((rc = ensure_device(pl))) return rc;
    PLAN_ENTER(stream);
    icv::KParams K;
    const icv::Layout* lay;
    if ((rc = fill_params(pl, m, ref_lo, ref_hi, lfc_clip, flags, const_cast<float*>(out), ldo,
                          const_cast<double*>(cell_median), nullptr, K, lay)))
        return rc;
    if (K.n_rows < 1) return ICV_OK;
    hipStream_t st = static_cast<hipStream_t>(stream);
    const int n_words = (pl->p.W + 63) / 64;
    const int64_t cs = thr ? chunksize : 1;
    auto* mk = reinterpret_cast<unsigned long long*>(mask);
    const icv::PackRing pr(pl->p.W);
    const bool ring = !knobs().no_mask_ring && pr.ok && (ldo & 3) == 0 && (reinterpret_cast<uintptr_t>(out) & 15) == 0 &&
                      (reinterpret_cast<uintptr_t>(mask) & 7) == 0;
    if (ring) {
        const int lds = pr.lds_bytes();
        const int64_t rounds = (K.n_rows + icv::kPmRows - 1) / icv::kPmRows;
        const unsigned gx = (unsigned)(rounds < pl->n_cu ? rounds : pl->n_cu);
        AsyncBuf ties;
        if (thr) HIP_TRY(ties.alloc((size_t)K.n_rows * icv::kPmPerRow * sizeof(unsigned long long), st));
        HIP_TRY(hipFuncSetAttribute(reinterpret_cast<const void*>(icv::k_thr_mask_ring),
                                    hipFuncAttributeMaxDynamicSharedMemorySize, icv::kPmLds));
        hipLaunchKernelGGL(icv::k_thr_mask_ring, dim3(gx), dim3(icv::kPmThreads), lds, st, K, thr, cs, row_phase, mk, n_words,
                           row_nnz, pl->d_tie_n, ties.as<unsigned long long>());
        if (thr) {
            dim3 tg(128), tb(256);
            const auto* tl = ties.as<unsigned long long>();
            if (m->dtype == ICV_F32) {
                if (m->format == ICV_DENSE)
                    hipLaunchKernelGGL((icv::k_thr_mask_ties<float, false>), tg, tb, 0, st, K, thr, cs, row_phase, mk, n_words, row_nnz, pl->d_tie_n, tl);
                else
                    hipLaunchKernelGGL((icv::k_thr_mask_ties<float, true>), tg, tb, 0, st, K, thr, cs, row_phase, mk, n_words, row_nnz, pl->d_tie_n, tl);
            } else {
                if (m->format == ICV_DENSE)
                    hipLaunchKernelGGL((icv::k_thr_mask_ties<double, false>), tg, tb, 0, st, K, thr, cs, row_phase, mk, n_words, row_nnz, pl->d_tie_n, tl);
                else
                    hipLaunchKernelGGL((icv::k_thr_mask_ties<double, true>), tg, tb, 0, st, K, thr, cs, row_phase, mk, n_words, row_nnz, pl->d_tie_n, tl);
            }
        }
        HIP_TRY(hipGetLastError());
        return ICV_OK;
    }
    dim3 grid((unsigned)K.n_rows), block(256);
    if (m->dtype == ICV_F32) {
        if (m->format == ICV_DENSE)
            hipLaunchKernelGGL((icv::k_thr_mask<float, false>), grid, block, 0, st, K, thr, cs, row_phase, mk, n_words, row_nnz);
        else
            hipLaunchKernelGGL((icv::k_thr_mask<float, true>), grid, block, 0, st, K, thr, cs, row_phase, mk, n_words, row_nnz);
    } else {
        if (m->format == ICV_DENSE)
            hipLaunchKernelGGL((icv::k_thr_mask<double, false>), grid, block, 0, st, K, thr, cs, row_phase, mk, n_words, row_nnz);
        else
            hipLaunchKernelGGL((icv::k_thr_mask<double, true>), grid, block, 0, st, K, thr, cs, row_phase, mk, n_words, row_nnz);
    }
    HIP_TRY(hipGetLastError());
    return ICV_OK;
}

int icv_threshold_pack(icv_plan_t pl, const icv_matrix* m, const void* ref_lo, const void* ref_hi, double lfc_clip,
                       int32_t flags, const float* out, int64_t ldo, const double* cell_median, const double* thr,
                       int64_t chunksize, int64_t row_phase, int64_t* indptr, int32_t* indices, double* data,
                       int64_t capacity, void* stream) {
    int rc = check_matrix(pl, m);
    if (rc) return rc;
    PLAN_BUSY_GUARD(pl);
    if (!cell_median || !indptr || !indices || !data || capacity < 0 ||
        (thr && (chunksize < 1 || row_phase < 0 || row_phase >= chunksize)))
        return fail(ICV_ERR_INVALID, "bad threshold_pack arguments");
    if (pl->p.W > 320 * 64) return fail(ICV_ERR_UNSUPPORTED, "icv_threshold_pack: more than 20480 windows");
    const int n_words = (pl->p.W + 63) / 64;
    int rpw = icv::kPackWords / n_words;
    rpw = rpw < 1 ? 1 : (rpw > icv::kPackMaxRows ? icv::kPackMaxRows : rpw);
    if ((rc = ensure_device(pl))) return rc;
    PLAN_ENTER(stream);
    icv::KParams K;
    const icv::Layout* lay;
    if ((rc = fill_params(pl, m, ref_lo, ref_hi, lfc_clip, flags, const_cast<float*>(out), ldo,
                          const_cast<double*>(cell_median), nullptr, K, lay)))
        return rc;
    hipStream_t st = static_cast<hipStream_t>(stream);
    if (K.n_rows < 1) {
        HIP_TRY(hipMemsetAsync(indptr, 0, sizeof(int64_t), st));
        return ICV_OK;
    }
    if (K.n_rows > 0xffffffffll) return fail(ICV_ERR_UNSUPPORTED, "icv_threshold_pack: more than 2^32 rows per call");
    const int64_t n_tickets = (K.n_rows + rpw - 1) / rpw, n_groups = (n_tickets + 63) / 64;
    AsyncBuf ws;
    HIP_TRY(ws.alloc((size_t)(n_tickets + 2 * n_groups + 1) * sizeof(unsigned long long), st));
    HIP_TRY(hipMemsetAsync(ws.p, 0, (size_t)(n_tickets + 2 * n_groups + 1) * sizeof(unsigned long long), st));
    auto* status = ws.as<unsigned long long>();
    auto* gstat = status + n_tickets;
    auto* gacc = gstat + n_groups;
    auto* ticket = reinterpret_cast<unsigned int*>(gacc + n_groups);
    const int64_t cs = thr ? chunksize : 1;
    dim3 grid((unsigned)n_tickets), block(256);
#define ICV_PACK(TT, CC) \
    hipLaunchKernelGGL((icv::k_thr_pack<TT, CC>), grid, block, 0, st, K, thr, cs, row_phase, rpw, ticket, status, gstat, gacc, indptr, indices, data, capacity)
    if (m->dtype == ICV_F32) {
        if (m->format == ICV_DENSE) ICV_PACK(float, false);
        else ICV_PACK(float, true);
    } else {
        if (m->format == ICV_DENSE) ICV_PACK(double, false);
        else ICV_PACK(double, true);
    }
#undef ICV_PACK
    HIP_TRY(hipGetLastError());
    return ICV_OK;
}

int icv_pack_geometry(int32_t n_windows, icv_pack_info* info) {
    if (!info || n_windows < 1) return fail(ICV_ERR_INVALID, "bad pack_geometry arguments");
    const icv::PackRing pr(n_windows);
    const icv::FillRing fr(n_windows);
    info->rows_per_round = icv::kPmRows;
    info->mask_streamed = pr.ok ? 1 : 0;
    info->mask_ring_slots = pr.ok ? pr.n_slots : 0;
    info->mask_lds_bytes = pr.ok ? pr.lds_bytes() : 0;
    info->mask_loads_in_flight = pr.ok ? (pr.n_slots - 1) * pr.per_loader : 0;
    info->fill_streamed = fr.ok ? 1 : 0;
    info->fill_ring_slots = fr.ok ? fr.n_slots : 0;
    info->fill_lds_bytes = fr.ok ? fr.lds_bytes() : 0;
    info->fill_loads_in_flight = fr.ok ? (fr.n_slots - 1) * (fr.per_loader + fr.n_extra) : 0;
    info->fill_stage_entries = fr.ok ? fr.cap : 0;
    return ICV_OK;
}

int icv_row_offsets(const int64_t* row_nnz, int64_t n_rows, int64_t* indptr, void* stream) {
    if ((!row_nnz && n_rows > 0) || !indptr || n_rows < 0) return fail(ICV_ERR_INVALID, "bad row_offsets arguments");
    hipStream_t st = static_cast<hipStream_t>(stream);
    const unsigned nb = (unsigned)((n_rows + icv::kScanBlock - 1) / icv::kScanBlock);
    AsyncBuf sums;
    HIP_TRY(sums.alloc((size_t)(nb ? nb : 1) * sizeof(int64_t), st));
    if (nb > 1) hipLaunchKernelGGL(icv::k_row_block_sums, dim3(nb), dim3(1024), 0, st, row_nnz, n_rows, sums.as<int64_t>());
    hipLaunchKernelGGL(icv::k_row_offsets, dim3(nb ? nb : 1), dim3(1024), 0, st, row_nnz, n_rows, sums.as<int64_t>(), indptr);
    HIP_TRY(hipGetLastError());
    return ICV_OK;
}

int icv_csr_fill_masked(const float* x, int64_t n_rows, int32_t n_cols, int64_t ld, const uint64_t* mask,
                        const int64_t* indptr, int32_t* indices, double* data, void* stream) {
    if (!x || !mask || !indptr || !indices || !data || n_cols < 0 || ld < n_cols)
        return fail(ICV_ERR_INVALID, "bad csr_fill_masked arguments");
    if (n_rows < 1) return ICV_OK;
    hipStream_t st = static_cast<hipStream_t>(stream);
    const icv::FillRing fr(n_cols);
    if (!knobs().no_fill_ring && fr.ok && (ld & 3) == 0 && (reinterpret_cast<uintptr_t>(x) & 15) == 0 &&
        (reinterpret_cast<uintptr_t>(mask) & 7) == 0) {
        const int n_cu = current_cu_count();
        const int64_t rounds = (n_rows + icv::kPmRows - 1) / icv::kPmRows;
        const unsigned gx = (unsigned)(rounds < n_cu ? rounds : n_cu);
        HIP_TRY(hipFuncSetAttribute(reinterpret_cast<const void*>(icv::k_csr_fill_ring),
                                    hipFuncAttributeMaxDynamicSharedMemorySize, icv::kPmLds));
        hipLaunchKernelGGL(icv::k_csr_fill_ring, dim3(gx), dim3(icv::kPmThreads), fr.lds_bytes(), st, x, n_rows, n_cols, ld,
                           reinterpret_cast<const unsigned long long*>(mask), indptr, indices, data);
        HIP_TRY(hipGetLastError());
        return ICV_OK;
    }
    hipLaunchKernelGGL(icv::k_csr_fill_masked, dim3((unsigned)((n_rows + 3) / 4)), dim3(256), 0, st, x, n_rows, n_cols, ld,
                       reinterpret_cast<const unsigned long long*>(mask), (n_cols + 63) / 64, indptr, indices, data);
    HIP_TRY(hipGetLastError());
    return ICV_OK;
}

int icv_csr_count(const float* x, int64_t n_rows, int32_t n_cols, int64_t ld, int64_t* row_nnz, void* stream) {
    if (!x || !row_nnz || n_cols < 0 || ld < n_cols) return fail(ICV_ERR_INVALID, "bad csr_count arguments");
    if (n_rows < 1) return ICV_OK;
    hipLaunchKernelGGL(icv::k_csr_count, dim3((unsigned)((n_rows + 3) / 4)), dim3(256), 0,
                       static_cast<hipStream_t>(stream), x, n_rows, n_cols, ld, row_nnz);
    HIP_TRY(hipGetLastError());
    return ICV_OK;
}

int icv_csr_fill(const float* x, int64_t n_rows, int32_t n_cols, int64_t ld, const int64_t* indptr, int32_t* indices,
                 double* data, void* stream) {
    if (!x || !indptr || !indices || !data || n_cols < 0 || ld < n_cols)
        return fail(ICV_ERR_INVALID, "bad csr_fill arguments");
    if (n_rows < 1) return ICV_OK;
    hipLaunchKernelGGL(icv::k_csr_fill, dim3((unsigned)((n_rows + 3) / 4)), dim3(256), 0,
                       static_cast<hipStream_t>(stream), x, n_rows, n_cols, ld, indptr, indices, data);
    HIP_TRY(hipGetLastError());
    return ICV_OK;
}

}

namespace {
struct GramWork {
    char* buf = nullptr;
    ~GramWork() { (void)hipFree(buf); }
};

template <bool DIST, bool SYM>
int launch_gram(hipStream_t st, GramWork& w, const float* z, int kz, const double* norm,
                const std::vector<icv::GramSuper>& supers, int64_t row_end, int64_t col_end, float* c_dir,
                int64_t ld_dir, float* c_mir, int64_t ld_mir) {
    if (supers.empty()) return ICV_OK;
    HIP_TRY(hipMalloc((void**)&w.buf, supers.size() * sizeof(icv::GramSuper)));
    HIP_TRY(hipMemcpyAsync(w.buf, supers.data(), supers.size() * sizeof(icv::GramSuper), hipMemcpyHostToDevice, st));
    icv::GramJob J;
    J.supers = reinterpret_cast<const icv::GramSuper*>(w.buf);
    J.n_supers = (int)supers.size();
    J.row_end = row_end;
    J.col_end = col_end;
    J.c_dir = c_dir;
    J.ld_dir = ld_dir;
// ... 1726 lines not shown
```

infercnvpy_amd/csrc/icv_kernel_chain.hpp:

```cpp
#pragma once
#include <hip/hip_runtime.h>
#include <cstdint>
#include "icv_kernels.hpp"

namespace icv {

constexpr int kChThreads = 1024;
constexpr int kChLoaders = 15;
constexpr int kChMaxLines = 4;
constexpr int kChLdsFull = 160 * 1024, kChLdsHalf = 80 * 1024;

typedef float chain_f2 __attribute__((ext_vector_type(2)));

__device__ __forceinline__ void chain_add(chain_f2& acc, const chain_f2 v) {
    asm volatile("v_pk_add_f32 %0, %0, %1" : "+v"(acc) : "v"(v));
}
__device__ __forceinline__ void chain_add(double& acc, const double v) {
    asm volatile("v_add_f64 %0, %0, %1" : "+v"(acc) : "v"(v));
}

template <typename T> struct ChainLane;
template <> struct ChainLane<float> { typedef chain_f2 type; };
template <> struct ChainLane<double> { typedef double type; };

// ... 133 lines not shown

template <typename T, int NL>
__device__ __forceinline__ void chain_rounds_var(const unsigned char* smem, int slot_bytes, int n_slots, int64_t n_rounds,
                                                 int lane, typename ChainLane<T>::type& a, int* ready, int* nch,
                                                 int* consumed) {
    typedef typename ChainLane<T>::type lane_t;
    constexpr int RB = 128 * NL;
    int slot_i = 0;
    const unsigned lds0 = (unsigned)(uintptr_t)smem + (unsigned)lane * 8u;
    for (int64_t k = 0; k < n_rounds; ++k) {
        while (__hip_atomic_load(ready + slot_i, __ATOMIC_ACQUIRE, __HIP_MEMORY_SCOPE_WORKGROUP) != (int)(k + 1))
            __builtin_amdgcn_s_sleep(1);
        const int n_chunks = __builtin_amdgcn_readfirstlane(nch[slot_i]);
        asm volatile("" ::: "memory");
        const unsigned p0 = lds0 + (unsigned)slot_i * (unsigned)slot_bytes;
        slot_i = slot_i + 1 == n_slots ? 0 : slot_i + 1;
        lane_t va[10], vb[10];
#define ICV_CH_VBODY(RBS, OP)                                              \
    ICV_CH_LOAD(RBS, va, p0);                                              \
    int c = 0;                                                             \
    for (; c + 2 < n_chunks; c += 2) {                                     \
        const unsigned p1 = p0 + (unsigned)((c + 1) * 10 * RB);            \
        ICV_CH_STEP(RBS, OP, a, vb, va, p1);                               \
        const unsigned p2 = p0 + (unsigned)((c + 2) * 10 * RB);            \
        ICV_CH_STEP(RBS, OP, a, va, vb, p2);                               \
    }                                                                      \
    if (c + 1 < n_chunks) {  \
        const unsigned p1 = p0 + (unsigned)((c + 1) * 10 * RB);            \
        ICV_CH_STEP(RBS, OP, a, vb, va, p1);                               \
        ICV_CH_ADDS(OP, a, vb);                                            \
    } else {                                                               \
        ICV_CH_ADDS(OP, a, va);                                            \
    }
        if constexpr (sizeof(T) == 4) {
            if constexpr (NL == 1) { ICV_CH_VBODY("128", "v_pk_add_f32") }
            else if constexpr (NL == 2) { ICV_CH_VBODY("256", "v_pk_add_f32") }
            else if constexpr (NL == 3) { ICV_CH_VBODY("384", "v_pk_add_f32") }
            else { ICV_CH_VBODY("512", "v_pk_add_f32") }
        } else {
            if constexpr (NL == 1) { ICV_CH_VBODY("128", "v_add_f64") }
            else if constexpr (NL == 2) { ICV_CH_VBODY("256", "v_add_f64") }
            else if constexpr (NL == 3) { ICV_CH_VBODY("384", "v_add_f64") }
            else { ICV_CH_VBODY("512", "v_add_f64") }
        }
#undef ICV_CH_VBODY
        asm volatile("s_waitcnt lgkmcnt(0)" ::: "memory");
        if (lane == 0) __hip_atomic_store(consumed, (int)(k + 1), __ATOMIC_RELEASE, __HIP_MEMORY_SCOPE_WORKGROUP);
    }
}

template <typename T, bool LIST>
__global__ void __launch_bounds__(kChThreads) k_colchain(const T* __restrict__ x, int64_t ld, int n_cols, int n_units,
                                                         int lds_bytes, const int32_t* __restrict__ sel, int64_t n_sel,
                                                         int64_t tail_row, T* __restrict__ acc) {
    extern __shared__ __attribute__((aligned(16))) unsigned char smem[];
    if (LIST && tail_row >= 0) {
        if ((int64_t)sel[n_sel - 1] == tail_row) n_sel -= 1;
        else tail_row = -1;
    }
    typedef typename ChainLane<T>::type lane_t;
    constexpr int EPL = 16 / (int)sizeof(T);
    constexpr int CPL = 8 / (int)sizeof(T);
    const int wave = __builtin_amdgcn_readfirstlane((int)(threadIdx.x >> 6));
    const int lane = threadIdx.x & 63;
    const int u = lds_bytes > kChLdsHalf ? 2 : 1;
    int unit0, nh;
    chain_tile_units(chain_tile_of_block((int)blockIdx.x, (int)gridDim.x), (int)gridDim.x, n_units, u, unit0, nh);
    const int c0 = unit0 * (64 / (int)sizeof(T));
    const ChainGeom g(nh, u);
    const int n_slots = lds_bytes / g.slot_bytes;
    int depth = n_slots - 1;
    if (depth * u > 15) depth = 15 / u;
    const int64_t n_rounds = (n_sel + g.round_rows - 1) / g.round_rows;
    const unsigned lds0 = (unsigned)(uintptr_t)smem;

    if (wave < kChLoaders) {
        const int q = lane / g.lpr;
        int col = c0 + (lane - q * g.lpr) * EPL;
        if (col >= n_cols) col = 0;
        const bool active = q < g.rpl;
        int issue_slot = 0;
        int32_t rs_next[2] = {0, 0};
        const auto fetch_list = [&](int64_t round) {
            if (LIST && round < n_rounds) {
                for (int j = 0; j < u; ++j) {
                    const int64_t r0 = round * g.round_rows + (j * kChLoaders + wave) * g.rpl;
                    int32_t rs = 0;
#pragma unroll
                    for (int i = 0; i < 16; ++i)
                        if (i < g.rpl) {
                            const int64_t ri = r0 + i < n_sel ? r0 + i : n_sel - 1;
                            const int32_t v = sel[ri];
                            if (q == i) rs = v;
                        }
                    rs_next[j] = rs;
                }
            }
        };
        const auto issue = [&](int64_t round) {
            const int32_t rs0 = rs_next[0], rs1 = rs_next[1];
            for (int j = 0; j < u; ++j) {
                int64_t r = round * g.round_rows + (j * kChLoaders + wave) * g.rpl + q;
                if (r >= n_sel) r = n_sel - 1;
                if (LIST) r = j ? rs1 : rs0;
                const unsigned dst = lds0 + (unsigned)issue_slot * (unsigned)g.slot_bytes +
                                     (unsigned)((j * kChLoaders + wave) * g.rpl) * (unsigned)g.row_bytes;
                if (active) lds_dma16(x + r * ld + col, dst);
            }
            issue_slot = issue_slot + 1 == n_slots ? 0 : issue_slot + 1;
            fetch_list(round + 1);
        };
        fetch_list(0);
        for (int64_t k = 0; k < depth - 1 && k < n_rounds; ++k) issue(k);
        for (int64_t k = 0; k < n_rounds; ++k) {
            if (k + depth - 1 < n_rounds) {
                issue(k + depth - 1);
                chain_wait_vmcnt((depth - 1) * u);
            } else {
                asm volatile("s_waitcnt vmcnt(0)" ::: "memory");
            }
            __builtin_amdgcn_s_barrier();
        }
    } else {
        const int col = lane * 8 < g.row_bytes ? c0 + lane * CPL : n_cols;
        lane_t a;
        if constexpr (sizeof(T) == 4) {
            a.x = col < n_cols ? acc[col] : 0.f;
            a.y = col + 1 < n_cols ? acc[col + 1] : 0.f;
        } else {
            a = col < n_cols ? acc[col] : 0.0;
        }
        const int rl = lane * 8 < g.row_bytes ? lane : 0;
        constexpr int L = kChLoaders;
        if (u == 2) {
            switch (nh) {
                case 1: chain_rounds<T, 1, 2 * L * 16>(smem, n_slots, n_rounds, n_sel, rl, a); break;
                case 2: chain_rounds<T, 2, 2 * L * 8>(smem, n_slots, n_rounds, n_sel, rl, a); break;
                case 3: chain_rounds<T, 3, 2 * L * 5>(smem, n_slots, n_rounds, n_sel, rl, a); break;
                case 4: chain_rounds<T, 4, 2 * L * 4>(smem, n_slots, n_rounds, n_sel, rl, a); break;
                case 5: chain_rounds<T, 5, 2 * L * 3>(smem, n_slots, n_rounds, n_sel, rl, a); break;
                case 6: chain_rounds<T, 6, 2 * L * 2>(smem, n_slots, n_rounds, n_sel, rl, a); break;
                case 7: chain_rounds<T, 7, 2 * L * 2>(smem, n_slots, n_rounds, n_sel, rl, a); break;
                default: chain_rounds<T, 8, 2 * L * 2>(smem, n_slots, n_rounds, n_sel, rl, a); break;
            }
        } else {
            switch (nh) {
                case 2: chain_rounds<T, 2, L * 8>(smem, n_slots, n_rounds, n_sel, rl, a); break;
                case 4: chain_rounds<T, 4, L * 4>(smem, n_slots, n_rounds, n_sel, rl, a); break;
                case 6: chain_rounds<T, 6, L * 2>(smem, n_slots, n_rounds, n_sel, rl, a); break;
                default: chain_rounds<T, 8, L * 2>(smem, n_slots, n_rounds, n_sel, rl, a); break;
            }
        }
        if (tail_row >= 0) {
            const T* xr = x + tail_row * ld;
            if constexpr (sizeof(T) == 4) {
                chain_f2 v;
                v.x = col < n_cols ? xr[col] : 0.f;
                v.y = col + 1 < n_cols ? xr[col + 1] : 0.f;
                chain_add(a, v);
            } else {
                chain_add(a, col < n_cols ? xr[col] : 0.0);
            }
        }
        if constexpr (sizeof(T) == 4) {
            if (col < n_cols) acc[col] = a.x;
            if (col + 1 < n_cols) acc[col + 1] = a.y;
        } else {
            if (col < n_cols) acc[col] = a;
        }
    }
}

struct ChainLaunch {
    int n_lines, grid, lds_bytes, n_units, dense_grid;
    ChainLaunch(int n_cols, int esz, int n_cu) {
        n_lines = (int)(((int64_t)n_cols * esz + 127) / 128);
        n_units = (int)(((int64_t)n_cols * esz + 63) / 64);
        if (n_lines <= kChMaxLines * n_cu) {
            grid = n_lines < n_cu ? n_lines : n_cu;
            lds_bytes = kChLdsFull;
        } else {
            grid = (n_lines + kChMaxLines - 1) / kChMaxLines;
            lds_bytes = grid <= n_cu ? kChLdsFull : kChLdsHalf;
        }
        if (grid < 1) grid = 1;
        dense_grid = lds_bytes == kChLdsFull ? (n_units < n_cu ? n_units : n_cu) : grid;
        if (dense_grid < 1) dense_grid = 1;
    }
};


constexpr int kCcRows = 60;
constexpr int kCcBlock = 32;
#ifndef ICV_CC_TABLE_ROW_MAJOR
#define ICV_CC_TABLE_ROW_MAJOR 1
#endif
__host__ __device__ inline int64_t cc_bounds_index(int64_t i, int t, int n_tiles) {
#if ICV_CC_TABLE_ROW_MAJOR
    return i * (int64_t)(n_tiles + 1) + t;
#else
    return ((i / kCcBlock) * (int64_t)(n_tiles + 1) + t) * kCcBlock + (i % kCcBlock);
#endif
}

template <bool LIST>
__global__ void __launch_bounds__(256) k_csr_tile_bounds(const int64_t* __restrict__ indptr,
                                                         const int32_t* __restrict__ indices,
                                                         const int32_t* __restrict__ sel, int64_t n_sel,
                                                         const uint16_t* __restrict__ line_tile, int esz_shift,
                                                         int n_tiles, uint32_t* __restrict__ bounds) {
    const int wave = threadIdx.x >> 6, lane = threadIdx.x & 63;
    for (int r = wave; r < kCcBlock; r += 4) {
        const int64_t i = (int64_t)blockIdx.x * kCcBlock + r;
        if (i >= n_sel) break;
        const int64_t row = LIST ? sel[i] : i;
        const int64_t e0 = indptr[row];
        const int64_t len = indptr[row + 1] - e0;
// ... 312 lines not shown
```

infercnvpy_amd/csrc/icv_kernels.hpp:

```cpp
#pragma once
#include <hip/hip_runtime.h>
#include <cstdint>

namespace icv {

constexpr int NT = 512;
constexpr int NWAVE = NT / 64;

struct KParams {
    const void* values;
    const int64_t* indptr;
    const int32_t* indices;
    int64_t n_rows;
    int64_t ld;
    int32_t n_cols;
    int32_t vec_ok;
    const void* ref_lo;
    const void* ref_hi;
    const void* zrow;
    int64_t zrow_bytes;
    int32_t bounded;
    int32_t trunc;
    double cap;
    const int32_t* dst;
// ... 177 lines not shown
}
template <int CTRL>
__device__ __forceinline__ int dpp_move_i(int v) {
    return __builtin_amdgcn_mov_dpp(v, CTRL, 0xf, 0xf, true);
}
__device__ __forceinline__ double readlane_d(double v, int lane) {
    int lo = __builtin_amdgcn_readlane(__double2loint(v), lane);
    int hi = __builtin_amdgcn_readlane(__double2hiint(v), lane);
    return __hiloint2double(hi, lo);
}
__device__ __forceinline__ double wave_sum_dpp(double v) {
    v += dpp_move<0xB1>(v);
    v += dpp_move<0x4E>(v);
    v += dpp_move<0x141>(v);
    v += dpp_move<0x140>(v);
    return ((readlane_d(v, 0) + readlane_d(v, 16)) + readlane_d(v, 32)) + readlane_d(v, 48);
}
__device__ __forceinline__ int wave_scan_dpp(int v) {
    v += __builtin_amdgcn_update_dpp(0, v, 0x111, 0xf, 0xf, false);
    v += __builtin_amdgcn_update_dpp(0, v, 0x112, 0xf, 0xf, false);
    v += __builtin_amdgcn_update_dpp(0, v, 0x114, 0xf, 0xf, false);
    v += __builtin_amdgcn_update_dpp(0, v, 0x118, 0xf, 0xf, false);
    v += __builtin_amdgcn_update_dpp(0, v, 0x142, 0xa, 0xf, false);
    v += __builtin_amdgcn_update_dpp(0, v, 0x143, 0xc, 0xf, false);
    return v;
}
__device__ __forceinline__ double wave_min_dpp(double v) {
    double o;
    o = dpp_move<0xB1>(v); v = o < v ? o : v;
    o = dpp_move<0x4E>(v); v = o < v ? o : v;
    o = dpp_move<0x141>(v); v = o < v ? o : v;
    o = dpp_move<0x140>(v); v = o < v ? o : v;
    double a = readlane_d(v, 0), b = readlane_d(v, 16), c = readlane_d(v, 32), d = readlane_d(v, 48);
    a = b < a ? b : a;
    c = d < c ? d : c;
    return c < a ? c : a;
}
__device__ __forceinline__ double wave_max_dpp(double v) { return -wave_min_dpp(-v); }

template <typename T> struct Vec16;
template <> struct Vec16<float> { using type = float4; using itype = int4; static constexpr int N = 4; };
template <> struct Vec16<double> { using type = double2; using itype = int2; static constexpr int N = 2; };

template <typename T>
__device__ __forceinline__ T vget(const typename Vec16<T>::type& v, int i);
template <> __device__ __forceinline__ float vget<float>(const float4& v, int i) {
    return i == 0 ? v.x : i == 1 ? v.y : i == 2 ? v.z : v.w;
}
template <> __device__ __forceinline__ double vget<double>(const double2& v, int i) { return i == 0 ? v.x : v.y; }
__device__ __forceinline__ int iget(const int4& v, int i) { return i == 0 ? v.x : i == 1 ? v.y : i == 2 ? v.z : v.w; }
__device__ __forceinline__ int iget(const int2& v, int i) { return i == 0 ? v.x : v.y; }

template <typename T, bool CSR, int MAXB >
__global__ void __launch_bounds__(NT) k_smooth(const KParams P) {
    extern __shared__ __attribute__((aligned(16))) unsigned char smem[];
    T* row = reinterpret_cast<T*>(smem);
    double* S01 = reinterpret_cast<double*>(smem);
    double* win = P.win_scratch ? P.win_scratch + (int64_t)blockIdx.x * P.W
                                : reinterpret_cast<double*>(smem + P.win_off);
    Scratch* sc = reinterpret_cast<Scratch*>(smem + P.scratch_off);

    using V = typename Vec16<T>::type;
    using IV = typename Vec16<T>::itype;
    constexpr int VN = Vec16<T>::N;
    constexpr int U = 4;

    const int t = threadIdx.x;
    const int lane = t & 63, wave = t >> 6;
    const T cap = (T)P.cap;
    const T* ref_lo = static_cast<const T*>(P.ref_lo);
    const T* ref_hi = P.bounded ? static_cast<const T*>(P.ref_hi) : ref_lo;
    const int W = P.W, B = P.B, NB = P.NB;

    for (int i = t; i < P.n_pad; i += NT) row[P.pad_idx[i]] = T(0);
    __syncthreads();

    unsigned long long tlast = 0, tacc[5] = {0, 0, 0, 0, 0};
#define ICV_PHASE(i)                                              \
    if (P.dbg && t == 0) {                                        \
        unsigned long long now_ = __builtin_amdgcn_s_memtime();   \
        tacc[i] += now_ - tlast;                                  \
        tlast = now_;                                             \
    }
    if (P.dbg && t == 0) tlast = __builtin_amdgcn_s_memtime();

    const int64_t n_work = P.row_list ? (int64_t)*P.row_count : P.n_rows;
    for (int64_t work = blockIdx.x; work < n_work; work += gridDim.x) {
        const int64_t cell = P.row_list ? P.row_list[work] : work;
        if constexpr (!CSR) {
            const T* xrow = static_cast<const T*>(P.values) + cell * P.ld;
            int done = 0;
            if (P.vec_ok) {
                const int nvec = P.n_cols / VN;
                const V* xv = reinterpret_cast<const V*>(xrow);
                const IV* dv = reinterpret_cast<const IV*>(P.dst);
                const V* lov = reinterpret_cast<const V*>(ref_lo);
                const V* hiv = reinterpret_cast<const V*>(ref_hi);
                for (int base = 0; base < nvec; base += NT * U) {
                    V x[U];
#pragma unroll
                    for (int u = 0; u < U; ++u) {
                        int i = base + u * NT + t;
                        if (i < nvec) x[u] = xv[i];
                    }
#pragma unroll
                    for (int u = 0; u < U; ++u) {
                        int i = base + u * NT + t;
// ... 180 lines not shown
                int ctot = 0;
                double mtot = __builtin_inf();
#pragma unroll
                for (int i = 0; i < NWAVE; ++i) {
                    ctot += sc->ired[0][i];
                    double m2 = sc->dred[1][0][i];
                    mtot = m2 < mtot ? m2 : mtot;
                }
                const double b = (ctot > k1 + 1) ? a : mtot;
                med = (a + b) / 2.0;
            }
        }

        ICV_PHASE(3)
        double sum = 0.0, sq = 0.0;
        float* orow = P.out + cell * P.ldo;
        for (int j = t; j < W; j += NT) {
            const double y = win[j] - med;
            orow[j] = (float)y;
            if (P.win_out) P.win_out[cell * P.win_ld + j] = win[j];
            sum = sum + y;
            sq = fma(y, y, sq);
        }
        sum = wave_sum_dpp(sum);
        sq = wave_sum_dpp(sq);
        if (lane == 0) {
            sc->dred[2][0][wave] = sum;
            sc->dred[2][1][wave] = sq;
        }
        __syncthreads();
        if (t == 0) {
            double s = 0.0, q = 0.0;
#pragma unroll
            for (int i = 0; i < NWAVE; ++i) {
                s += sc->dred[2][0][i];
                q += sc->dred[2][1][i];
            }
            P.cell_stats[2 * cell] = s;
            P.cell_stats[2 * cell + 1] = q;
            P.cell_median[cell] = med;
        }
        if constexpr (MAXB > 0) {
            __syncthreads();
            for (int i = t; i < P.n_pad; i += NT) row[P.pad_idx[i]] = T(0);
        }
        __syncthreads();
        ICV_PHASE(4)
    }
    if (P.dbg && t == 0)
        for (int i = 0; i < 5; ++i) atomicAdd(P.dbg + i, tacc[i]);
#undef ICV_PHASE
}

typedef unsigned int u32x4 __attribute__((ext_vector_type(4)));
typedef unsigned int u32x2 __attribute__((ext_vector_type(2)));
__device__ __forceinline__ __amdgpu_buffer_rsrc_t make_rsrc(const void* p, unsigned bytes) {
    return __builtin_amdgcn_make_buffer_rsrc(const_cast<void*>(p), 0, (int)bytes, 0x00020000);
}

template <typename T>
__global__ void k_zero_row(KParams P, T* zrow, int n_alloc) {
    int i = blockIdx.x * blockDim.x + threadIdx.x;
    if (i >= n_alloc) return;
    T v = T(0);
    if (i < P.Gp) {
        int g = P.src[i];
        if (g >= 0) {
            const T* lo = static_cast<const T*>(P.ref_lo);
            const T* hi = P.bounded ? static_cast<const T*>(P.ref_hi) : lo;
            v = centre_clip<T>(T(0), lo[g], hi[g], (T)P.cap, P.bounded, P.trunc);
        }
    }
    zrow[i] = v;
}

__global__ void __launch_bounds__(256) k_csr_prepare(const KParams P, int64_t k0, int64_t k1, uint16_t* pos16,
                                                     float* cvals) {
    const float* lo = static_cast<const float*>(P.ref_lo);
    const float* hi = P.bounded ? static_cast<const float*>(P.ref_hi) : lo;
    const float* vals = static_cast<const float*>(P.values);
    for (int64_t k = k0 + (int64_t)blockIdx.x * 256 + threadIdx.x; k < k1; k += (int64_t)gridDim.x * 256) {
        const int g = P.indices[k];
        pos16[k] = P.dst16[g];
        cvals[k] = centre_clip<float>(vals[k], lo[g], hi[g], (float)P.cap, P.bounded, P.trunc);
    }
}

__global__ void __launch_bounds__(256) k_chunk_thr(const double* stats, int64_t n_rows, int64_t chunksize,
                                                   int64_t row_phase, int n_windows, double dyn, double* thr) {
    __shared__ double ss[256], sq[256];
    const int64_t k = blockIdx.x;
    int64_t r0 = k * chunksize - row_phase, r1 = r0 + chunksize;
    if (r0 < 0) r0 = 0;
    if (r1 > n_rows) r1 = n_rows;
    double s = 0.0, q = 0.0;
    for (int64_t r = r0 + threadIdx.x; r < r1; r += 256) {
        s += stats[2 * r];
        q += stats[2 * r + 1];
    }
    ss[threadIdx.x] = s;
    sq[threadIdx.x] = q;
    __syncthreads();
    for (int o = 128; o > 0; o >>= 1) {
        if ((int)threadIdx.x < o) {
            ss[threadIdx.x] += ss[threadIdx.x + o];
            sq[threadIdx.x] += sq[threadIdx.x + o];
        }
        __syncthreads();
    }
    if (threadIdx.x == 0) {
        const double n = (double)(r1 - r0) * (double)n_windows;
        const double mean = ss[0] / n;
        double var = (sq[0] - ss[0] * mean) / n;
        if (var < 0.0) var = 0.0;
        thr[k] = dyn * sqrt(var);
    }
}

__global__ void __launch_bounds__(256) k_chunk_thr_part(const double* chunk_part, int n_part, const double* hb_stats,
                                                        int64_t n_rows, int64_t chunksize, int64_t row_phase,
                                                        int n_windows, double dyn, double* thr) {
    __shared__ double ss[256], sq[256];
    const int64_t k = blockIdx.x;
    int64_t r0 = k * chunksize - row_phase, r1 = r0 + chunksize;
    if (r0 < 0) r0 = 0;
    if (r1 > n_rows) r1 = n_rows;
    double s = 0.0, q = 0.0;
    const double2* part = reinterpret_cast<const double2*>(chunk_part) + k * n_part;
    for (int i = threadIdx.x; i < n_part; i += 256) {
        const double2 v = part[i];
        s += v.x;
        q += v.y;
    }
    for (int64_t r = r0 + threadIdx.x; r < r1; r += 256) {
        s += hb_stats[2 * r];
        q += hb_stats[2 * r + 1];
    }
    ss[threadIdx.x] = s;
    sq[threadIdx.x] = q;
    __syncthreads();
    for (int o = 128; o > 0; o >>= 1) {
        if ((int)threadIdx.x < o) {
            ss[threadIdx.x] += ss[threadIdx.x + o];
            sq[threadIdx.x] += sq[threadIdx.x + o];
        }
        __syncthreads();
    }
    if (threadIdx.x == 0) {
        const double n = (double)(r1 - r0) * (double)n_windows;
        const double mean = ss[0] / n;
        double var = (sq[0] - ss[0] * mean) / n;
        if (var < 0.0) var = 0.0;
        thr[k] = dyn * sqrt(var);
    }
}

__device__ __forceinline__ int thr_compare(float a, float thf) {
    if (!(thf > 0.0f) || !(a == a)) return 1;
    const int d = __float_as_int(a) - __float_as_int(thf);
    return d < -1 ? -1 : (d > 1 ? 1 : 0);
}

template <typename T, bool CSR>
__device__ double value_at(const KParams& P, int64_t cell, int pp) {
    const int g = P.src[pp];
    if (g < 0) return 0.0;
    const T* ref_lo = static_cast<const T*>(P.ref_lo);
    const T* ref_hi = P.bounded ? static_cast<const T*>(P.ref_hi) : ref_lo;
    T x = T(0);
    if constexpr (!CSR) {
        x = static_cast<const T*>(P.values)[cell * P.ld + g];
    } else {
        int64_t lo = P.indptr[cell], hi = P.indptr[cell + 1];
        while (lo < hi) {
            const int64_t mid = (lo + hi) >> 1;
            if (P.indices[mid] < g) lo = mid + 1;
            else hi = mid;
        }
        if (lo < P.indptr[cell + 1] && P.indices[lo] == g) x = static_cast<const T*>(P.values)[lo];
    }
    return (double)centre_clip<T>(x, ref_lo[g], ref_hi[g], (T)P.cap, P.bounded, P.trunc);
}

template <typename F>
__device__ double window_canonical(const KParams& P, int j, F val) {
    const int ln = P.w_len[j];
    double acc;
    if (P.B > 1) {
        const int B = P.B;
        acc = window_from_blocks(ln, B, [&](int m, double& s0, double& s1) {
            s0 = 0.0;
            s1 = 0.0;
            for (int r = 0; r < B; ++r) block_accumulate(val(m * B + r), r, s0, s1);
        });
    } else {
        acc = window_direct(ln, val);
    }
    return finish_window(acc, ln, P.pyr_den, P.pyr_rcp, P.w_denom[j]);
}

constexpr int kTieBuf = 2048;

template <typename T, bool CSR>
__global__ void __launch_bounds__(256) k_apply_thr(const KParams P, const double* thr, int64_t chunksize,
                                                   int64_t row_phase) {
    __shared__ int tie_n;
// ... 676 lines not shown
    if (row >= n_rows) return;
    const float* xr = x + row * ld;
    int c = 0;
    for (int j = threadIdx.x & 63; j < n_cols; j += 64) c += (xr[j] != 0.0f) ? 1 : 0;
    c = wave_sum_i(c);
    if ((threadIdx.x & 63) == 0) row_nnz[row] = c;
}

__global__ void __launch_bounds__(256) k_csr_fill(const float* x, int64_t n_rows, int n_cols, int64_t ld,
                                                  const int64_t* indptr, int32_t* indices, double* data) {
    const int64_t row = (int64_t)blockIdx.x * 4 + (threadIdx.x >> 6);
    if (row >= n_rows) return;
    const int lane = threadIdx.x & 63;
    const float* xr = x + row * ld;
    int64_t base = indptr[row];
    for (int j0 = 0; j0 < n_cols; j0 += 64) {
        const int j = j0 + lane;
        const float v = j < n_cols ? xr[j] : 0.0f;
        const bool nz = v != 0.0f;
        const unsigned long long m = __builtin_amdgcn_ballot_w64(nz);
        if (nz) {
            const int pos = __builtin_amdgcn_mbcnt_hi((unsigned)(m >> 32), __builtin_amdgcn_mbcnt_lo((unsigned)m, 0));
            indices[base + pos] = j;
            data[base + pos] = (double)v;
        }
        base += __popcll(m);
    }
}

template <typename T>
__global__ void __launch_bounds__(256) k_csr_row_abs_sum(const T* data, const int64_t* indptr, int64_t n_rows,
                                                         double* row_sum) {
    const int64_t row = (int64_t)blockIdx.x * 4 + (threadIdx.x >> 6);
    if (row >= n_rows) return;
    double acc = 0.0;
    const int64_t e = indptr[row + 1];
    for (int64_t k = indptr[row] + (threadIdx.x & 63); k < e; k += 64) acc += fabs((double)data[k]);
    acc = wave_sum(acc);
    if ((threadIdx.x & 63) == 0) row_sum[row] = acc;
}

constexpr int kScanPer = 4;
constexpr int kScanBlock = 1024 * kScanPer;
__device__ __forceinline__ long long block_sum_1024(long long s, long long* wsum) {
    s = (long long)wave_sum_u64((unsigned long long)s);
    __syncthreads();
    if ((threadIdx.x & 63) == 0) wsum[threadIdx.x >> 6] = s;
    __syncthreads();
    long long tot = 0;
#pragma unroll
    for (int w = 0; w < 16; ++w) tot += wsum[w];
    return tot;
}
__global__ void __launch_bounds__(1024) k_row_block_sums(const int64_t* __restrict__ row_nnz, int64_t n_rows,
                                                         int64_t* __restrict__ block_sums) {
    __shared__ long long wsum[16];
    const int64_t r0 = (int64_t)blockIdx.x * kScanBlock + (int64_t)kScanPer * threadIdx.x;
    long long s = 0;
#pragma unroll
    for (int k = 0; k < kScanPer; ++k) s += r0 + k < n_rows ? row_nnz[r0 + k] : 0;
    const long long tot = block_sum_1024(s, wsum);
    if (threadIdx.x == 0) block_sums[blockIdx.x] = tot;
}
__global__ void __launch_bounds__(1024) k_row_offsets(const int64_t* __restrict__ row_nnz, int64_t n_rows,
                                                      const int64_t* __restrict__ block_sums,
                                                      int64_t* __restrict__ indptr) {
    __shared__ long long wsum[16];
    const int t = threadIdx.x, lane = t & 63, wave = t >> 6;
    const int64_t r0 = (int64_t)blockIdx.x * kScanBlock + (int64_t)kScanPer * t;
    long long v[kScanPer], s = 0;
#pragma unroll
    for (int k = 0; k < kScanPer; ++k) {
        v[k] = r0 + k < n_rows ? row_nnz[r0 + k] : 0;
        s += v[k];
    }
    long long before = 0;
    for (int b = t; b < (int)blockIdx.x; b += 1024) before += block_sums[b];
    before = block_sum_1024(before, wsum);
    long long incl = s;
#pragma unroll
    for (int o = 1; o < 64; o <<= 1) {
        const unsigned lo = (unsigned)__shfl_up((int)(unsigned)incl, o);
        const unsigned hi = (unsigned)__shfl_up((int)(unsigned)((unsigned long long)incl >> 32), o);
        if (lane >= o) incl += (long long)(((unsigned long long)hi << 32) | lo);
    }
    __syncthreads();
    if (lane == 63) wsum[wave] = incl;
    __syncthreads();
    for (int w = 0; w < wave; ++w) before += wsum[w];
    long long run = before + incl - s;
    if (blockIdx.x == 0 && t == 0) indptr[0] = 0;
#pragma unroll
    for (int k = 0; k < kScanPer; ++k) {
        run += v[k];
        if (r0 + k < n_rows) indptr[r0 + k + 1] = run;
    }
}

__global__ void __launch_bounds__(256) k_csr_fill_masked(const float* x, int64_t n_rows, int n_cols, int64_t ld,
                                                         const unsigned long long* mask, int n_words,
                                                         const int64_t* indptr, int32_t* indices, double* data) {
    const int64_t row = (int64_t)blockIdx.x * 4 + (threadIdx.x >> 6);
    if (row >= n_rows) return;
    const int lane = threadIdx.x & 63;
    const float* xr = x + row * ld;
    const unsigned long long* mrow = mask + row * (int64_t)n_words;
    int64_t base = indptr[row];
    for (int w0 = 0; w0 < n_words; w0 += 64) {
        const int nw = n_words - w0 < 64 ? n_words - w0 : 64;
        const unsigned long long mine = lane < nw ? mrow[w0 + lane] : 0ull;
        const int cnt = __popcll(mine);
        const int incl = wave_scan_dpp(cnt);
        const int excl = incl - cnt;
        const unsigned mlo = (unsigned)mine, mhi = (unsigned)(mine >> 32);
        for (int w = 0; w < nw; ++w) {
            const unsigned lo = (unsigned)__builtin_amdgcn_readlane((int)mlo, w), hi = (unsigned)__builtin_amdgcn_readlane((int)mhi, w);
            if ((lo | hi) == 0u) continue;
            const unsigned long long m = ((unsigned long long)hi << 32) | lo;
            const int off = __builtin_amdgcn_readlane(excl, w);
            if ((m >> lane) & 1ull) {
                const int j = (w0 + w) * 64 + lane;
                const int pos = off + __builtin_amdgcn_mbcnt_hi(hi, __builtin_amdgcn_mbcnt_lo(lo, 0));
                indices[base + pos] = j;
                data[base + pos] = (double)xr[j];
            }
        }
        base += __builtin_amdgcn_readlane(incl, 63);
    }
}

}
```

infercnvpy_amd/tl/_infercnv.py:

```python
from __future__ import annotations

import logging
import os
import sys
import threading
import time as _time
from collections.abc import Sequence

import numpy as np
import scipy.sparse as sp

from .. import _engine, _lib
from .._plan import GenePlan

log = logging.getLogger("infercnvpy_amd")

_MIN_CHUNKS_PER_DEVICE = 4
_MIN_ROWS_PER_DEVICE = 50_000


def _reference_groups(obs, reference_key, reference_cat):
    obs_col = obs[reference_key]
    if isinstance(reference_cat, str):
        reference_cat = [reference_cat]
# ... 189 lines not shown

def _is_real_anndata(adata):
    mod = type(adata).__module__ or ""
    return mod == "anndata" or mod.startswith("anndata.")


def _repeat_rows(rows, cats):
    if cats is None:
        return rows
    labels = cats.tolist()
    if len(set(labels)) == len(labels):
        return rows
    first = {c: i for i, c in reversed(list(enumerate(labels)))}
    return [rows[first[c]] for c in labels]


def _infercnv_resident(var, obs, dm, *, reference_key, reference_cat, reference, lfc_clip, window_size, step,
                       dynamic_threshold, exclude_chromosomes, chunksize, calculate_gene_values, mean_order, tm):
    torch = _engine._torch()
    t_start = _time.perf_counter()
    dev = dm._keep[0].device.index
    n_obs, n_vars = dm.shape
    with torch.cuda.device(dev):
        ent, plan = _checkout_plan(var["chromosome"].to_numpy(), var["start"].to_numpy(), window_size, step,
                                   exclude_chromosomes, dev)
        try:
            if plan.n_without_position:
                log.warning(f"Skipped {plan.n_without_position} genes because they don't have a genomic position annotated. ")
            is_csr = dm.format == _lib.ICV_CSR
            np_dtype = np.float32 if dm.dtype == torch.float32 else np.float64
            flags = 0
            if reference is not None:
                given = np.asarray(reference)
                if given.ndim == 1:
                    given = given[np.newaxis, :]
                if given.shape[1] != n_vars:
                    raise ValueError("Reference must match the number of genes in AnnData. ")
                if np.result_type(np_dtype, given.dtype) != np_dtype:
                    raise ValueError("a device-resident matrix needs a reference of its own (or a narrower) dtype: "
                                     "numpy would promote the subtraction (pass the matrix as float64)")
                ref = torch.from_numpy(np.ascontiguousarray(given.astype(np_dtype))).cuda()
            else:
                groups = cats = None
                if reference_key is None or reference_cat is None:
                    log.warning("Using mean of all cells as reference. For better results, provide either "
                                "`reference`, or both `reference_key` and `reference_cat`. ")
                    counts = [n_obs]
                else:
                    groups, counts, cats = _reference_groups(obs, reference_key, reference_cat)
                if mean_order == "float64":
                    sums = _engine.column_sums(dm, groups, len(counts))
                    cnt = torch.as_tensor(np.asarray(counts, dtype=np.float64)).cuda()
                    rows = list((sums / cnt[:, None]).to(dm.dtype))
                else:
                    rows = []
                    for gi, n_g in enumerate(counts):
                        sel = None if groups is None else np.nonzero(groups == gi)[0]
                        acc = _engine.column_chain(dm, None, sel, int(n_g))
                        rows.append(_engine.chain_mean(acc, int(n_g), is_csr))
                ref = torch.stack(_repeat_rows(rows, cats))
            if ref.shape[0] == 1:
                ref_lo, ref_hi = ref[0].contiguous(), None
            else:
                ref_lo, ref_hi = ref.min(dim=0).values.contiguous(), ref.max(dim=0).values.contiguous()
            free_b = _engine.free_hbm_bytes()
            per_row = 16 * plan.n_windows + 64 + (8 * (n_vars + plan.n_windows) if calculate_gene_values else 0)
            if calculate_gene_values:
                free_b = max(free_b - 8 * n_vars * n_obs, free_b // 8)
            piece = max(chunksize, int(0.4 * free_b // per_row) // chunksize * chunksize)
            parts = []
            genes = torch.empty((n_obs, n_vars), dtype=torch.float64, device="cuda") if calculate_gene_values else None
            for r0 in range(0, max(n_obs, 1), piece):
                r1 = min(n_obs, r0 + piece)
                res = _engine.run_hot_path(plan, dm, ref_lo, ref_hi, lfc_clip=lfc_clip,
                                           dynamic_threshold=dynamic_threshold, chunksize=chunksize, flags=flags,
                                           row0=r0, row1=r1, apply=False, windows=calculate_gene_values)
                parts.append(_engine.threshold_csr(plan, dm, ref_lo, ref_hi, res, lfc_clip=lfc_clip,
                                                   chunksize=chunksize, flags=flags, row0=r0, row1=r1))
                if calculate_gene_values and r1 > r0:
                    _engine.gene_values_from_windows(plan, res.windows, thr=res.thr, chunksize=chunksize,
                                                     out=genes[r0:r1])
                del res
            x_cnv = parts[0] if len(parts) == 1 else _engine.concat_packed(parts)
            tm["kernel"] = plan.last_kernel()
            tm["devices"] = [dev]
            tm["pieces"] = len(parts)
            tm["total"] = _time.perf_counter() - t_start
            chr_pos = dict(plan.chr_pos)
        finally:
            _checkin_plan(ent, plan)
    return chr_pos, x_cnv, genes


def _check_var(var, var_names):
    if not var_names.is_unique:
        raise ValueError("Ensure your var_names are unique!")
    if {"chromosome", "start", "end"} - set(var.columns) != set():
        raise ValueError(
            "Genomic positions not found. There need to be `chromosome`, `start`, and `end` columns in `adata.var`. ")


def _check_mean_order(mean_order):
    if mean_order not in ("reference", "float64"):
        raise ValueError("mean_order must be 'reference' (numpy's / scipy's evaluation order) or 'float64'")


def infercnv_device(
    X,
    var,
    obs=None,
    *,
    reference_key: str | None = None,
    reference_cat: None | str | Sequence[str] = None,
# ... 406 lines not shown
```

Baseline: 32.09 million.

## Fuse threshold computation into hand-back kernel, merge mean, and fuse offset scan

Several launch-overhead reductions. The chunk-threshold computation is folded into a new hand-back kernel that uses a last-block atomic to finish the thresholds and reset stats, replacing per-call memsets. The column mean is computed inside the colchain kernel, so no separate mean launch is needed. The row-offset scan is fused into the threshold-mask step, and the row-count reset moves into a tiny kernel instead of a memset. This removes kernel launches and memsets per call, in exchange for more complex cross-block synchronisation and persistent zeroed-state invariants that could break if a call aborts.

New measurement: 32.31 million, median of 5. Within noise of the previous version (+0.7%).

```diff
diff --git a/include/infercnv_hip.h b/include/infercnv_hip.h
--- a/include/infercnv_hip.h
+++ b/include/infercnv_hip.h
@@ -84,6 +84,7 @@
 int icv_colsum_pairwise(const void *xt, int32_t dtype, int64_t n_rows, int32_t n_cols, int64_t ld, void *sums,
                         void *stream);
 int icv_colchain_mean(const void *acc, int32_t dtype, int32_t n_cols, int64_t count, void *mean, void *stream);
+int icv_colchain_means(const icv_matrix *m, void *mean, void *stream);
 int icv_colmean_csc(const void *values, int32_t dtype, const int64_t *colptr, const int32_t *row_idx, int32_t n_cols,
                     const int32_t *row_group, int32_t group, double scale, void *mean, void *stream);
 
@@ -156,6 +157,10 @@
 int icv_csr_fill_masked(const float *x, int64_t n_rows, int32_t n_cols, int64_t ld, const uint64_t *mask,
                         const int64_t *indptr, int32_t *indices, double *data, void *stream);
 int icv_row_offsets(const int64_t *row_nnz, int64_t n_rows, int64_t *indptr, void *stream);
+int icv_threshold_offsets(icv_plan_t plan, const icv_matrix *m, const void *ref_lo, const void *ref_hi,
+                          double lfc_clip, int32_t flags, const float *out, int64_t ldo, const double *cell_median,
+                          const double *thr, int64_t chunksize, int64_t row_phase, uint64_t *mask, int64_t *row_nnz,
+                          int64_t *indptr, void *stream);
 
 int icv_threshold_pack(icv_plan_t plan, const icv_matrix *m, const void *ref_lo, const void *ref_hi, double lfc_clip,
                        int32_t flags, const float *out, int64_t ldo, const double *cell_median, const double *thr,
diff --git a/infercnvpy_amd/_engine.py b/infercnvpy_amd/_engine.py
--- a/infercnvpy_amd/_engine.py
+++ b/infercnvpy_amd/_engine.py
@@ -237,6 +237,17 @@
     out = torch.empty_like(acc)
     _lib.check(lib.icv_colchain_mean(_ptr(acc), _lib.ICV_F32 if acc.dtype == torch.float32 else _lib.ICV_F64,
                                      acc.numel(), int(count), _ptr(out), _stream_ptr(torch)))
+    return out
+
+
+def column_means(dm: DeviceMatrix):
+    torch = _torch()
+    lib = _lib.load()
+    if dm.format != _lib.ICV_DENSE or dm.shape[0] < 1:
+        raise ValueError("column_means: a dense matrix with at least one row")
+    out = torch.empty(dm.shape[1], dtype=dm.dtype, device="cuda")
+    m = dm.c_struct(0, None)
+    _lib.check(lib.icv_colchain_means(C.byref(m), _ptr(out), _stream_ptr(torch)))
     return out
 
 
@@ -637,7 +648,7 @@
 
 
 def threshold_mask(plan: GenePlan, dm: DeviceMatrix, ref_lo, ref_hi, res, *, lfc_clip, chunksize, row_phase=0,
-                   flags=0, row0=0, row1=None):
+                   flags=0, row0=0, row1=None, indptr=None):
     torch = _torch()
     lib = _lib.load()
     rows = res.out.shape[0]
@@ -645,10 +656,13 @@
     mask = torch.empty((rows, n_words), dtype=torch.int64, device="cuda")
     counts = torch.empty(rows, dtype=torch.int64, device="cuda")
     m = dm.c_struct(row0, row1)
-    _lib.check(lib.icv_threshold_mask(
-        plan.handle, C.byref(m), _ptr(ref_lo), _ptr(ref_hi), float(lfc_clip), int(flags), _ptr(res.out),
-        res.out.stride(0), _ptr(res.cell_median), _ptr(res.thr), int(chunksize), int(row_phase), _ptr(mask),
-        _ptr(counts), _stream_ptr(torch)))
+    args = (plan.handle, C.byref(m), _ptr(ref_lo), _ptr(ref_hi), float(lfc_clip), int(flags), _ptr(res.out),
+            res.out.stride(0), _ptr(res.cell_median), _ptr(res.thr), int(chunksize), int(row_phase), _ptr(mask),
+            _ptr(counts))
+    if indptr is None:
+        _lib.check(lib.icv_threshold_mask(*args, _stream_ptr(torch)))
+    else:
+        _lib.check(lib.icv_threshold_offsets(*args, _ptr(indptr), _stream_ptr(torch)))
     return PackedRows(res.out, mask, counts, res.thr)
 
 
@@ -717,14 +731,13 @@
     if single_pass and W <= 20480:
         return threshold_pack(plan, dm, ref_lo, ref_hi, res, lfc_clip=lfc_clip, chunksize=chunksize,
                               row_phase=row_phase, flags=flags, row0=row0, row1=row1, capacity=capacity)
+    indptr = torch.empty(rows + 1, dtype=torch.int64, device="cuda")
     part = threshold_mask(plan, dm, ref_lo, ref_hi, res, lfc_clip=lfc_clip, chunksize=chunksize, row_phase=row_phase,
-                          flags=flags, row0=row0, row1=row1)
+                          flags=flags, row0=row0, row1=row1, indptr=indptr)
     cap = rows * W if capacity is None else max(int(capacity), rows * W)
-    indptr = torch.empty(rows + 1, dtype=torch.int64, device="cuda")
     indices = torch.empty(max(cap, 1), dtype=torch.int32, device="cuda")
     data = torch.empty(max(cap, 1), dtype=torch.float64, device="cuda")
     st = _stream_ptr(torch)
-    _lib.check(lib.icv_row_offsets(_ptr(part.counts), rows, _ptr(indptr), st))
     if rows:
         _lib.check(lib.icv_csr_fill_masked(_ptr(part.out), rows, W, part.out.stride(0), _ptr(part.mask), _ptr(indptr),
                                            _ptr(indices), _ptr(data), st))
diff --git a/infercnvpy_amd/_lib.py b/infercnvpy_amd/_lib.py
--- a/infercnvpy_amd/_lib.py
+++ b/infercnvpy_amd/_lib.py
@@ -19,11 +19,11 @@
 EXPORTS = (
     "icv_plan_create", "icv_plan_destroy", "icv_plan_get_info", "icv_plan_chr_pos", "icv_plan_window_table",
     "icv_plan_last_kernel", "icv_plan_se_tables", "icv_plan_gene_runs",
-    "icv_colsum", "icv_colchain", "icv_colsum_pairwise", "icv_colchain_mean", "icv_colmean_csc", "icv_infercnv_smooth", "icv_chunk_thresholds", "icv_apply_threshold", "icv_infercnv_run",
+    "icv_colsum", "icv_colchain", "icv_colsum_pairwise", "icv_colchain_mean", "icv_colchain_means", "icv_colmean_csc", "icv_infercnv_smooth", "icv_chunk_thresholds", "icv_apply_threshold", "icv_infercnv_run",
     "icv_infercnv_run_windows", "icv_gene_values_from_windows",
     "icv_colchain_blocks_workspace", "icv_colchain_blocks_sums", "icv_colchain_blocks_records", "icv_colchain_blocks_scan",
     "icv_profile_begin", "icv_profile_collect",
-    "icv_gene_values", "icv_csr_count", "icv_csr_fill", "icv_threshold_mask", "icv_csr_fill_masked", "icv_row_offsets", "icv_pack_geometry", "icv_threshold_pack", "icv_corr_iqr",
+    "icv_gene_values", "icv_csr_count", "icv_csr_fill", "icv_threshold_mask", "icv_threshold_offsets", "icv_csr_fill_masked", "icv_row_offsets", "icv_pack_geometry", "icv_threshold_pack", "icv_corr_iqr",
     "icv_pairwise_sqeuclidean", "icv_ward_linkage", "icv_pairwise_sqeuclidean_tiles",
     "icv_ward_create", "icv_ward_destroy", "icv_ward_merge", "icv_ward_gather", "icv_ward_scatter", "icv_ward_scan", "icv_ward_pack_nn",
     "icv_ward_unpack_nn", "icv_ward_pairs", "icv_ward_round_pairs", "icv_ward_finish", "icv_row_abs_sum", "icv_csr_row_abs_sum", "icv_group_sums", "icv_csr_check", "icv_csr_densify", "icv_gram_f64", "icv_project", "icv_host_dense_row_nnz", "icv_host_dense_pack", "icv_host_dense_pack_fused", "icv_csr_scatter_dense", "icv_last_error", "icv_version",
@@ -93,6 +93,7 @@
     lib.icv_colchain.argtypes = [P(Matrix), vp, i64, dbl, vp, vp]
     lib.icv_colsum_pairwise.argtypes = [vp, i32, i64, i32, i64, vp, vp]
     lib.icv_colchain_mean.argtypes = [vp, i32, i32, i64, vp, vp]
+    lib.icv_colchain_means.argtypes = [P(Matrix), vp, vp]
     lib.icv_colmean_csc.argtypes = [vp, i32, vp, vp, i32, vp, i32, dbl, vp, vp]
     lib.icv_infercnv_smooth.argtypes = [vp, P(Matrix), vp, vp, dbl, i32, vp, i64, vp, vp, vp]
     lib.icv_chunk_thresholds.argtypes = [vp, i64, i64, i64, i32, dbl, vp, vp]
@@ -114,6 +115,7 @@
     lib.icv_threshold_mask.argtypes = [vp, P(Matrix), vp, vp, dbl, i32, vp, i64, vp, vp, i64, i64, vp, vp, vp]
     lib.icv_threshold_pack.argtypes = [vp, P(Matrix), vp, vp, dbl, i32, vp, i64, vp, vp, i64, i64, vp, vp, vp, i64, vp]
     lib.icv_row_offsets.argtypes = [vp, i64, vp, vp]
+    lib.icv_threshold_offsets.argtypes = [vp, P(Matrix), vp, vp, dbl, i32, vp, i64, vp, vp, i64, i64, vp, vp, vp, vp]
     lib.icv_pack_geometry.argtypes = [i32, P(PackInfo)]
     lib.icv_csr_fill_masked.argtypes = [vp, i64, i32, i64, vp, vp, vp, vp, vp]
     lib.icv_corr_iqr.argtypes = [vp, i64, i32, i64, P(C.c_double), vp]
diff --git a/infercnvpy_amd/csrc/icv_api.hip b/infercnvpy_amd/csrc/icv_api.hip
--- a/infercnvpy_amd/csrc/icv_api.hip
+++ b/infercnvpy_amd/csrc/icv_api.hip
@@ -120,6 +120,10 @@
     int64_t* d_row_list = nullptr;
     int* d_row_count = nullptr;
     int64_t row_list_cap = 0;
+    bool defer_hand_back = false;
+    int hand_back_left = 0;
+    bool hb_stats_zero = false;
+    bool ring_attr_set = false;
     bool prof_deferred = false;
     std::vector<hipEvent_t> prof_events;
     double* d_win_scratch = nullptr;
@@ -249,8 +253,9 @@
     HIP_TRY(up(p.pad_idx.data(), p.pad_idx.size() * 4, (void**)&pl->d_pad));
     HIP_TRY(up(p.w_pack.data(), p.w_pack.size() * 4, (void**)&pl->d_wpack));
     {
-        const unsigned zeros[2] = {0u, 0u};
+        const unsigned zeros[8] = {0u, 0u, 0u, 0u, 0u, 0u, 0u, 0u};
         HIP_TRY(up(zeros, sizeof(zeros), (void**)&pl->d_tie_n));
+        HIP_TRY(up(zeros, sizeof(int), (void**)&pl->d_row_count));
     }
     HIP_TRY(up(p.cov_col.data(), p.cov_col.size() * 4, (void**)&pl->d_cov_col));
     HIP_TRY(up(p.cov_j0.data(), p.cov_j0.size() * 4, (void**)&pl->d_cov_j0));
@@ -476,7 +481,7 @@
            ((p.B == 10 && p.window == 100 && p.x16_fine == 4096) || (p.B == 5 && p.window == 250 && p.x16_fine == 1024));
 }
 
-int hand_back_workspace(icv_plan_t pl, icv::KParams& K, hipStream_t st) {
+int hand_back_workspace(icv_plan_t pl, icv::KParams& K) {
     if (pl->row_list_cap < K.n_rows) {
         (void)hipFree(pl->d_row_list);
         pl->d_row_list = nullptr;
@@ -492,15 +497,19 @@
         pl->cell_part_cap = K.n_rows;
     }
     K.cell_part = pl->d_cell_part;
-    if (!pl->d_row_count) HIP_TRY(hipMalloc((void**)&pl->d_row_count, sizeof(int)));
-    HIP_TRY(hipMemsetAsync(pl->d_row_count, 0, sizeof(int), st));
     K.row_list = pl->d_row_list;
     K.row_count = pl->d_row_count;
     return ICV_OK;
 }
 
+__global__ void k_reset_count(int* count) { *count = 0; }
+
 int launch_hand_back(icv_plan_t pl, const icv::KParams& K, hipStream_t st, bool csr) {
     const icv::Plan& p = pl->p;
+    if (pl->defer_hand_back) {
+        pl->hand_back_left = csr ? 2 : 1;
+        return ICV_OK;
+    }
     icv::KParams G = K;
     G.win_off = p.lay32.win_off;
     G.scratch_off = p.lay32.scratch_off;
@@ -514,6 +523,28 @@
     int64_t g2 = pl->n_cu;
     if (g2 > K.n_rows) g2 = K.n_rows;
     hipLaunchKernelGGL(gk, dim3((unsigned)g2), dim3(icv::NT), p.lay32.total, st, G);
+    hipLaunchKernelGGL(k_reset_count, dim3(1), dim3(1), 0, st, pl->d_row_count);
+    HIP_TRY(hipGetLastError());
+    return ICV_OK;
+}
+
+int launch_hand_back_thr(icv_plan_t pl, const icv::KParams& K, hipStream_t st, bool csr, int n_wg, int n_wave,
+                         unsigned wave_mask, int64_t n_chunks, double dyn, double* thr) {
+    const icv::Plan& p = pl->p;
+    icv::KParams G = K;
+    G.win_off = p.lay32.win_off;
+    G.scratch_off = p.lay32.scratch_off;
+    G.dbg = nullptr;
+    const int need = (p.NB + icv::kThreads - 1) / icv::kThreads;
+    void (*gk)(const icv::KParams, int, int, unsigned, int64_t, double, double*, unsigned*);
+    if (csr) gk = need <= 4 ? icv::k_hand_back_thr<true, 4> : icv::k_hand_back_thr<true, 8>;
+    else gk = need <= 4 ? icv::k_hand_back_thr<false, 4> : icv::k_hand_back_thr<false, 8>;
+    const int lds = p.lay32.total > 4096 ? p.lay32.total : 4096;
+    HIP_TRY(hipFuncSetAttribute(reinterpret_cast<const void*>(gk), hipFuncAttributeMaxDynamicSharedMemorySize, lds));
+    int64_t g2 = pl->n_cu;
+    if (g2 > K.n_rows) g2 = K.n_rows;
+    hipLaunchKernelGGL(gk, dim3((unsigned)g2), dim3(icv::NT), lds, st, G, n_wg, n_wave, wave_mask, n_chunks, dyn, thr,
+                       pl->d_tie_n + 5);
     HIP_TRY(hipGetLastError());
     return ICV_OK;
 }
@@ -567,7 +598,7 @@
     hipLaunchKernelGGL(icv::k_se_wtab, dim3((unsigned)((n_wt + 255) / 256)), dim3(256), 0, st, K,
                        static_cast<const float*>(pl->d_zrow), pl->d_se_w0, pl->d_se_w1, wt_guard.as<icv::u32x4>(),
                        g_guard.as<double>(), K.sd_r);
-    if (int rc = hand_back_workspace(pl, K, st)) return rc;
+    if (int rc = hand_back_workspace(pl, K)) return rc;
     int64_t grid = se_grid(pl, K.n_rows);
     if (grid < 1) {
         if (kernel_done) HIP_TRY(hipEventRecord(kernel_done, st));
@@ -649,7 +680,7 @@
                                    const_cast<uint16_t*>(K.pos16), const_cast<float*>(K.cvals));
         }
         K.hist_off = p.ws_hist_off;
-        if (int rc = hand_back_workspace(pl, K, st)) return rc;
+        if (int rc = hand_back_workspace(pl, K)) return rc;
     }
     int per_cu = icv::kLdsLimit / lds;
     if (per_cu > 4) per_cu = 4;
@@ -887,7 +918,8 @@
 }
 
 template <typename T>
-int colchain_dense(const icv_matrix* m, const int32_t* rows, int64_t n_sel, T* acc, hipStream_t st) {
+int colchain_dense(const icv_matrix* m, const int32_t* rows, int64_t n_sel, T* acc, hipStream_t st, T* mean = nullptr,
+                   T denom = T(1)) {
     const icv::ChainLaunch L(m->n_cols, (int)sizeof(T), current_cu_count());
     constexpr int EPL = 16 / (int)sizeof(T);
     int64_t tail = -1, n_dma = n_sel;
@@ -895,12 +927,12 @@
         tail = m->n_rows - 1;
         if (!rows) n_dma = n_sel - 1;
     }
-    typedef void (*kern_t)(const T*, int64_t, int, int, int, const int32_t*, int64_t, int64_t, T*);
+    typedef void (*kern_t)(const T*, int64_t, int, int, int, const int32_t*, int64_t, int64_t, T*, T*, T);
     const kern_t kern = rows ? (kern_t)icv::k_colchain<T, true> : (kern_t)icv::k_colchain<T, false>;
     HIP_TRY(hipFuncSetAttribute(reinterpret_cast<const void*>(kern), hipFuncAttributeMaxDynamicSharedMemorySize,
                                 icv::kChLdsFull));
     hipLaunchKernelGGL(kern, dim3(L.dense_grid), dim3(icv::kChThreads), L.lds_bytes, st, (const T*)m->values, m->ld,
-                       m->n_cols, L.n_units, L.lds_bytes, rows, n_dma, tail, acc);
+                       m->n_cols, L.n_units, L.lds_bytes, rows, n_dma, tail, acc, mean, denom);
     HIP_TRY(hipGetLastError());
     return ICV_OK;
 }
@@ -1293,6 +1325,18 @@
                                : colchain_dense<double>(m, rows, n_sel, (double*)acc, st);
 }
 
+int icv_colchain_means(const icv_matrix* m, void* mean, void* stream) {
+    if (!m || !mean) return fail(ICV_ERR_INVALID, "bad colchain_means arguments");
+    if (m->dtype != ICV_F32 && m->dtype != ICV_F64) return fail(ICV_ERR_INVALID, "dtype must be ICV_F32 or ICV_F64");
+    if (m->format != ICV_DENSE) return fail(ICV_ERR_INVALID, "icv_colchain_means: dense input only");
+    if (m->n_rows < 1) return fail(ICV_ERR_INVALID, "icv_colchain_means: no rows");
+    if (m->n_cols == 0) return ICV_OK;
+    hipStream_t st = static_cast<hipStream_t>(stream);
+    return m->dtype == ICV_F32
+               ? colchain_dense<float>(m, nullptr, m->n_rows, nullptr, st, (float*)mean, (float)m->n_rows)
+               : colchain_dense<double>(m, nullptr, m->n_rows, nullptr, st, (double*)mean, (double)m->n_rows);
+}
+
 int icv_colchain_mean(const void* acc, int32_t dtype, int32_t n_cols, int64_t count, void* mean, void* stream) {
     if (!acc || !mean || count < 1 || n_cols < 0) return fail(ICV_ERR_INVALID, "bad colchain_mean arguments");
     hipStream_t st = static_cast<hipStream_t>(stream);
@@ -1419,6 +1463,7 @@
             pl->hb_stats_cap = 0;
             HIP_TRY(hipMalloc((void**)&pl->d_hb_stats, (size_t)m->n_rows * 2 * sizeof(double)));
             pl->hb_stats_cap = m->n_rows;
+            pl->hb_stats_zero = false;
         }
         K.cell_stats = pl->d_hb_stats;
         const int64_t se_slots = ((int64_t)pl->n_cu * (icv::kLdsLimit / icv::kSeLds)) * icv::NWAVE;
@@ -1434,13 +1479,24 @@
                 HIP_TRY(hipMalloc((void**)&pl->d_chunk_part, (size_t)(n_chunks * n_part) * 2 * sizeof(double)));
                 pl->chunk_part_cap = n_chunks * n_part;
             }
-            HIP_TRY(hipMemsetAsync(pl->d_chunk_part, 0, (size_t)(n_chunks * n_part) * 2 * sizeof(double), st));
-            HIP_TRY(hipMemsetAsync(pl->d_hb_stats, 0, (size_t)m->n_rows * 2 * sizeof(double), st));
             K.chunk_part = pl->d_chunk_part;
             K.chunksize = cs_eff;
             K.row_phase = ph_eff;
         }
     }
+    const bool fused_thr = do_thr && chunk_mode;
+    if (fused_thr && !pl->hb_stats_zero) {
+        HIP_TRY(hipMemsetAsync(pl->d_hb_stats, 0, (size_t)pl->hb_stats_cap * 2 * sizeof(double), st));
+        pl->hb_stats_zero = true;
+    } else if (!fused_thr && K.cell_stats == pl->d_hb_stats) {
+        pl->hb_stats_zero = false;
+    }
+    struct DeferGuard {
+        icv_plan_t pl;
+        ~DeferGuard() { pl->defer_hand_back = false; }
+    } defer_guard{pl};
+    pl->defer_hand_back = fused_thr;
+    pl->hand_back_left = 0;
     EventSet evs;
     hipEvent_t* ev = evs.ev;
     const bool deferred = !prof && pl->prof_deferred;
@@ -1452,19 +1508,33 @@
     bool ev1_done = false;
     if ((rc = launch_smooth(pl, m, K, *lay, st, timed ? ev[1] : nullptr, &ev1_done))) return rc;
     if (timed && !ev1_done) HIP_TRY(hipEventRecord(ev[1], st));
-    if (do_thr && chunk_mode) {
-        int64_t n_slots;
+    pl->defer_hand_back = false;
+    if (fused_thr && !pl->hand_back_left) {
+        pl->hb_stats_zero = false;
+        rc = icv_chunk_thresholds(K.cell_stats, m->n_rows, chunksize, row_phase, pl->p.W, dynamic_threshold, thr, stream);
+        if (rc) return rc;
+    } else if (fused_thr) {
+        int64_t n_wg;
+        int n_wave;
+        unsigned wave_mask;
         if (m->format == ICV_CSR) {
-            n_slots = se_grid(pl, m->n_rows) * icv::NWAVE;
+            n_wg = se_grid(pl, m->n_rows);
+            n_wave = icv::NWAVE;
+            wave_mask = (1u << icv::NWAVE) - 1u;
         } else {
-            int64_t gx = pl->n_cu;
-            if (gx > m->n_rows) gx = m->n_rows;
-            n_slots = gx * icv::XWAVE;
-        }
-        hipLaunchKernelGGL(icv::k_chunk_thr_part, dim3((unsigned)n_chunks), dim3(256), 0, st, pl->d_chunk_part,
-                           (int)n_slots, pl->d_hb_stats, m->n_rows, chunksize, row_phase, pl->p.W,
-                           dynamic_threshold, thr);
-        HIP_TRY(hipGetLastError());
+            n_wg = pl->n_cu;
+            if (n_wg > m->n_rows) n_wg = m->n_rows;
+            n_wave = icv::XWAVE;
+            wave_mask = 0u;
+            for (int t = 0; t < icv::XT; ++t)
+                if ((pl->p.x16_wdesc[t] >> 24) & 1u) wave_mask |= 1u << (t >> 6);
+        }
+        K.row_list = pl->d_row_list;
+        K.row_count = pl->d_row_count;
+        K.cell_part = pl->d_cell_part;
+        if ((rc = launch_hand_back_thr(pl, K, st, pl->hand_back_left == 2, (int)n_wg, n_wave, wave_mask, n_chunks,
+                                       dynamic_threshold, thr)))
+            return rc;
     } else if (do_thr && m->n_rows > 0) {
         rc = icv_chunk_thresholds(K.cell_stats, m->n_rows, chunksize, row_phase, pl->p.W, dynamic_threshold, thr,
                                   stream);
@@ -1634,9 +1704,43 @@
     return gene_from_windows(pl, b_win.as<double>(), W, n, thr, chunksize, row_phase, gene_out, ldg, st);
 }
 
-int icv_threshold_mask(icv_plan_t pl, const icv_matrix* m, const void* ref_lo, const void* ref_hi, double lfc_clip,
-                       int32_t flags, const float* out, int64_t ldo, const double* cell_median, const double* thr,
-                       int64_t chunksize, int64_t row_phase, uint64_t* mask, int64_t* row_nnz, void* stream) {
+}
+
+namespace {
+int ring_attributes(icv_plan_t pl) {
+    if (pl->ring_attr_set) return ICV_OK;
+    HIP_TRY(hipFuncSetAttribute(reinterpret_cast<const void*>(icv::k_thr_mask_ring),
+                                hipFuncAttributeMaxDynamicSharedMemorySize, icv::kPmLds));
+    pl->ring_attr_set = true;
+    return ICV_OK;
+}
+
+int fill_ring_attributes() {
+    static std::atomic<bool> done[64];
+    int dev = 0;
+    HIP_TRY(hipGetDevice(&dev));
+    const bool known = dev >= 0 && dev < 64;
+    if (known && done[dev].load(std::memory_order_acquire)) return ICV_OK;
+    HIP_TRY(hipFuncSetAttribute(reinterpret_cast<const void*>(icv::k_csr_fill_ring),
+                                hipFuncAttributeMaxDynamicSharedMemorySize, icv::kPmLds));
+    if (known) done[dev].store(true, std::memory_order_release);
+    return ICV_OK;
+}
+
+int row_offsets(const int64_t* row_nnz, int64_t n_rows, int64_t* indptr, hipStream_t st) {
+    const unsigned nb = (unsigned)((n_rows + icv::kScanBlock - 1) / icv::kScanBlock);
+    AsyncBuf sums;
+    HIP_TRY(sums.alloc((size_t)(nb ? nb : 1) * sizeof(int64_t), st));
+    if (nb > 1) hipLaunchKernelGGL(icv::k_row_block_sums, dim3(nb), dim3(1024), 0, st, row_nnz, n_rows, sums.as<int64_t>());
+    hipLaunchKernelGGL(icv::k_row_offsets, dim3(nb ? nb : 1), dim3(1024), 0, st, row_nnz, n_rows, sums.as<int64_t>(), indptr);
+    HIP_TRY(hipGetLastError());
+    return ICV_OK;
+}
+
+int threshold_mask(icv_plan_t pl, const icv_matrix* m, const void* ref_lo, const void* ref_hi, double lfc_clip,
+                   int32_t flags, const float* out, int64_t ldo, const double* cell_median, const double* thr,
+                   int64_t chunksize, int64_t row_phase, uint64_t* mask, int64_t* row_nnz, int64_t* indptr,
+                   void* stream) {
     int rc = check_matrix(pl, m);
     if (rc) return rc;
     PLAN_BUSY_GUARD(pl);
@@ -1649,8 +1753,8 @@
     if ((rc = fill_params(pl, m, ref_lo, ref_hi, lfc_clip, flags, const_cast<float*>(out), ldo,
                           const_cast<double*>(cell_median), nullptr, K, lay)))
         return rc;
-    if (K.n_rows < 1) return ICV_OK;
     hipStream_t st = static_cast<hipStream_t>(stream);
+    if (K.n_rows < 1) return indptr ? row_offsets(row_nnz, 0, indptr, st) : ICV_OK;
     const int n_words = (pl->p.W + 63) / 64;
     const int64_t cs = thr ? chunksize : 1;
     auto* mk = reinterpret_cast<unsigned long long*>(mask);
@@ -1663,8 +1767,7 @@
         const unsigned gx = (unsigned)(rounds < pl->n_cu ? rounds : pl->n_cu);
         AsyncBuf ties;
         if (thr) HIP_TRY(ties.alloc((size_t)K.n_rows * icv::kPmPerRow * sizeof(unsigned long long), st));
-        HIP_TRY(hipFuncSetAttribute(reinterpret_cast<const void*>(icv::k_thr_mask_ring),
-                                    hipFuncAttributeMaxDynamicSharedMemorySize, icv::kPmLds));
+        if ((rc = ring_attributes(pl))) return rc;
         hipLaunchKernelGGL(icv::k_thr_mask_ring, dim3(gx), dim3(icv::kPmThreads), lds, st, K, thr, cs, row_phase, mk, n_words,
                            row_nnz, pl->d_tie_n, ties.as<unsigned long long>());
         if (thr) {
@@ -1683,7 +1786,7 @@
             }
         }
         HIP_TRY(hipGetLastError());
-        return ICV_OK;
+        return indptr ? row_offsets(row_nnz, K.n_rows, indptr, st) : ICV_OK;
     }
     dim3 grid((unsigned)K.n_rows), block(256);
     if (m->dtype == ICV_F32) {
@@ -1698,7 +1801,26 @@
             hipLaunchKernelGGL((icv::k_thr_mask<double, true>), grid, block, 0, st, K, thr, cs, row_phase, mk, n_words, row_nnz);
     }
     HIP_TRY(hipGetLastError());
-    return ICV_OK;
+    return indptr ? row_offsets(row_nnz, K.n_rows, indptr, st) : ICV_OK;
+}
+}
+
+extern "C" {
+
+int icv_threshold_mask(icv_plan_t pl, const icv_matrix* m, const void* ref_lo, const void* ref_hi, double lfc_clip,
+                       int32_t flags, const float* out, int64_t ldo, const double* cell_median, const double* thr,
+                       int64_t chunksize, int64_t row_phase, uint64_t* mask, int64_t* row_nnz, void* stream) {
+    return threshold_mask(pl, m, ref_lo, ref_hi, lfc_clip, flags, out, ldo, cell_median, thr, chunksize, row_phase, mask,
+                          row_nnz, nullptr, stream);
+}
+
+int icv_threshold_offsets(icv_plan_t pl, const icv_matrix* m, const void* ref_lo, const void* ref_hi, double lfc_clip,
+                          int32_t flags, const float* out, int64_t ldo, const double* cell_median, const double* thr,
+                          int64_t chunksize, int64_t row_phase, uint64_t* mask, int64_t* row_nnz, int64_t* indptr,
+                          void* stream) {
+    if (!indptr) return fail(ICV_ERR_INVALID, "bad threshold_offsets arguments");
+    return threshold_mask(pl, m, ref_lo, ref_hi, lfc_clip, flags, out, ldo, cell_median, thr, chunksize, row_phase, mask,
+                          row_nnz, indptr, stream);
 }
 
 int icv_threshold_pack(icv_plan_t pl, const icv_matrix* m, const void* ref_lo, const void* ref_hi, double lfc_clip,
@@ -1771,14 +1893,7 @@
 
 int icv_row_offsets(const int64_t* row_nnz, int64_t n_rows, int64_t* indptr, void* stream) {
     if ((!row_nnz && n_rows > 0) || !indptr || n_rows < 0) return fail(ICV_ERR_INVALID, "bad row_offsets arguments");
-    hipStream_t st = static_cast<hipStream_t>(stream);
-    const unsigned nb = (unsigned)((n_rows + icv::kScanBlock - 1) / icv::kScanBlock);
-    AsyncBuf sums;
-    HIP_TRY(sums.alloc((size_t)(nb ? nb : 1) * sizeof(int64_t), st));
-    if (nb > 1) hipLaunchKernelGGL(icv::k_row_block_sums, dim3(nb), dim3(1024), 0, st, row_nnz, n_rows, sums.as<int64_t>());
-    hipLaunchKernelGGL(icv::k_row_offsets, dim3(nb ? nb : 1), dim3(1024), 0, st, row_nnz, n_rows, sums.as<int64_t>(), indptr);
-    HIP_TRY(hipGetLastError());
-    return ICV_OK;
+    return row_offsets(row_nnz, n_rows, indptr, static_cast<hipStream_t>(stream));
 }
 
 int icv_csr_fill_masked(const float* x, int64_t n_rows, int32_t n_cols, int64_t ld, const uint64_t* mask,
@@ -1793,8 +1908,7 @@
         const int n_cu = current_cu_count();
         const int64_t rounds = (n_rows + icv::kPmRows - 1) / icv::kPmRows;
         const unsigned gx = (unsigned)(rounds < n_cu ? rounds : n_cu);
-        HIP_TRY(hipFuncSetAttribute(reinterpret_cast<const void*>(icv::k_csr_fill_ring),
-                                    hipFuncAttributeMaxDynamicSharedMemorySize, icv::kPmLds));
+        if (int rc = fill_ring_attributes()) return rc;
         hipLaunchKernelGGL(icv::k_csr_fill_ring, dim3(gx), dim3(icv::kPmThreads), fr.lds_bytes(), st, x, n_rows, n_cols, ld,
                            reinterpret_cast<const unsigned long long*>(mask), indptr, indices, data);
         HIP_TRY(hipGetLastError());
diff --git a/infercnvpy_amd/csrc/icv_kernel_chain.hpp b/infercnvpy_amd/csrc/icv_kernel_chain.hpp
--- a/infercnvpy_amd/csrc/icv_kernel_chain.hpp
+++ b/infercnvpy_amd/csrc/icv_kernel_chain.hpp
@@ -209,7 +209,8 @@
 template <typename T, bool LIST>
 __global__ void __launch_bounds__(kChThreads) k_colchain(const T* __restrict__ x, int64_t ld, int n_cols, int n_units,
                                                          int lds_bytes, const int32_t* __restrict__ sel, int64_t n_sel,
-                                                         int64_t tail_row, T* __restrict__ acc) {
+                                                         int64_t tail_row, T* __restrict__ acc, T* __restrict__ mean,
+                                                         T denom) {
     extern __shared__ __attribute__((aligned(16))) unsigned char smem[];
     if (LIST && tail_row >= 0) {
         if ((int64_t)sel[n_sel - 1] == tail_row) n_sel -= 1;
@@ -282,10 +283,10 @@
         const int col = lane * 8 < g.row_bytes ? c0 + lane * CPL : n_cols;
         lane_t a;
         if constexpr (sizeof(T) == 4) {
-            a.x = col < n_cols ? acc[col] : 0.f;
-            a.y = col + 1 < n_cols ? acc[col + 1] : 0.f;
-        } else {
-            a = col < n_cols ? acc[col] : 0.0;
+            a.x = !mean && col < n_cols ? acc[col] : 0.f;
+            a.y = !mean && col + 1 < n_cols ? acc[col + 1] : 0.f;
+        } else {
+            a = !mean && col < n_cols ? acc[col] : 0.0;
         }
         const int rl = lane * 8 < g.row_bytes ? lane : 0;
         constexpr int L = kChLoaders;
@@ -319,7 +320,14 @@
                 chain_add(a, col < n_cols ? xr[col] : 0.0);
             }
         }
-        if constexpr (sizeof(T) == 4) {
+        if (mean) {
+            if constexpr (sizeof(T) == 4) {
+                if (col < n_cols) mean[col] = a.x / denom;
+                if (col + 1 < n_cols) mean[col + 1] = a.y / denom;
+            } else {
+                if (col < n_cols) mean[col] = a / denom;
+            }
+        } else if constexpr (sizeof(T) == 4) {
             if (col < n_cols) acc[col] = a.x;
             if (col + 1 < n_cols) acc[col + 1] = a.y;
         } else {
diff --git a/infercnvpy_amd/csrc/icv_kernels.hpp b/infercnvpy_amd/csrc/icv_kernels.hpp
--- a/infercnvpy_amd/csrc/icv_kernels.hpp
+++ b/infercnvpy_amd/csrc/icv_kernels.hpp
@@ -253,7 +253,7 @@
 __device__ __forceinline__ int iget(const int2& v, int i) { return i == 0 ? v.x : v.y; }
 
 template <typename T, bool CSR, int MAXB >
-__global__ void __launch_bounds__(NT) k_smooth(const KParams P) {
+__device__ __forceinline__ void smooth_rows(const KParams& P) {
     extern __shared__ __attribute__((aligned(16))) unsigned char smem[];
     T* row = reinterpret_cast<T*>(smem);
     double* S01 = reinterpret_cast<double*>(smem);
@@ -540,6 +540,11 @@
 #undef ICV_PHASE
 }
 
+template <typename T, bool CSR, int MAXB >
+__global__ void __launch_bounds__(NT) k_smooth(const KParams P) {
+    smooth_rows<T, CSR, MAXB>(P);
+}
+
 typedef unsigned int u32x4 __attribute__((ext_vector_type(4)));
 typedef unsigned int u32x2 __attribute__((ext_vector_type(2)));
 __device__ __forceinline__ __amdgpu_buffer_rsrc_t make_rsrc(const void* p, unsigned bytes) {
@@ -640,6 +645,91 @@
         double var = (sq[0] - ss[0] * mean) / n;
         if (var < 0.0) var = 0.0;
         thr[k] = dyn * sqrt(var);
+    }
+}
+
+__device__ __forceinline__ void chunk_thr_from_parts(double* ss, int64_t k, const double* chunk_part, int n_wg, int n_wave,
+                                                     unsigned wave_mask, const double* hb_stats, int64_t n_rows,
+                                                     int64_t chunksize, int64_t row_phase, int n_windows, double dyn,
+                                                     double* thr) {
+    double* sq = ss + 256;
+    const int t = threadIdx.x;
+    int64_t r0 = k * chunksize - row_phase, r1 = r0 + chunksize;
+    if (r0 < 0) r0 = 0;
+    if (r1 > n_rows) r1 = n_rows;
+    if (t < 256) {
+        double s = 0.0, q = 0.0;
+        const int n_part = n_wg * n_wave;
+        const double2* part = reinterpret_cast<const double2*>(chunk_part) + k * n_part;
+        const int g_first = (int)(r0 % n_wg);
+        for (int i = t; i < n_part; i += 256) {
+            const int g = i / n_wave, w = i - g * n_wave;
+            const int d = g >= g_first ? g - g_first : g - g_first + n_wg;
+            if (!((wave_mask >> w) & 1u) || r0 + d >= r1) continue;
+            const double2 v = part[i];
+            s += v.x;
+            q += v.y;
+        }
+        if (hb_stats)
+            for (int64_t r = r0 + t; r < r1; r += 256) {
+                s += hb_stats[2 * r];
+                q += hb_stats[2 * r + 1];
+            }
+        ss[t] = s;
+        sq[t] = q;
+    }
+    __syncthreads();
+    for (int o = 128; o > 0; o >>= 1) {
+        if (t < o) {
+            ss[t] += ss[t + o];
+            sq[t] += sq[t + o];
+        }
+        __syncthreads();
+    }
+    if (t == 0) {
+        const double n = (double)(r1 - r0) * (double)n_windows;
+        const double mean = ss[0] / n;
+        double var = (sq[0] - ss[0] * mean) / n;
+        if (var < 0.0) var = 0.0;
+        thr[k] = dyn * sqrt(var);
+    }
+    __syncthreads();
+}
+
+template <bool CSR, int MAXB>
+__global__ void __launch_bounds__(NT) k_hand_back_thr(const KParams P, int n_wg, int n_wave, unsigned wave_mask,
+                                                      int64_t n_chunks, double dyn, double* thr, unsigned* done) {
+    extern __shared__ __attribute__((aligned(16))) unsigned char smem[];
+    const int n_hb = *P.row_count;
+    if (n_hb == 0) {
+        for (int64_t k = blockIdx.x; k < n_chunks; k += gridDim.x)
+            chunk_thr_from_parts(reinterpret_cast<double*>(smem), k, P.chunk_part, n_wg, n_wave, wave_mask, nullptr,
+                                 P.n_rows, P.chunksize, P.row_phase, P.W, dyn, thr);
+        return;
+    }
+    smooth_rows<float, CSR, MAXB>(P);
+    __syncthreads();
+    int* last = reinterpret_cast<int*>(smem);
+    if (threadIdx.x == 0) {
+        __threadfence();
+        *last = atomicAdd(done, 1u) == gridDim.x - 1;
+    }
+    __syncthreads();
+    const bool is_last = *last != 0;
+    __syncthreads();
+    if (!is_last) return;
+    __builtin_amdgcn_fence(__ATOMIC_ACQUIRE, "agent");
+    for (int64_t k = 0; k < n_chunks; ++k)
+        chunk_thr_from_parts(reinterpret_cast<double*>(smem), k, P.chunk_part, n_wg, n_wave, wave_mask, P.cell_stats,
+                             P.n_rows, P.chunksize, P.row_phase, P.W, dyn, thr);
+    for (int i = threadIdx.x; i < n_hb; i += NT) {
+        const int64_t r = P.row_list[i];
+        P.cell_stats[2 * r] = 0.0;
+        P.cell_stats[2 * r + 1] = 0.0;
+    }
+    if (threadIdx.x == 0) {
+        *P.row_count = 0;
+        *done = 0u;
     }
 }
 
@@ -1422,49 +1512,57 @@
     for (int w = 0; w < 16; ++w) tot += wsum[w];
     return tot;
 }
+__device__ __forceinline__ void row_block_sum(const int64_t* row_nnz, int64_t n_rows, int64_t* block_sums, unsigned blk,
+                                              long long* wsum) {
+    const int64_t r0 = (int64_t)blk * kScanBlock + (int64_t)kScanPer * threadIdx.x;
+    long long s = 0;
+#pragma unroll
+    for (int k = 0; k < kScanPer; ++k) s += r0 + k < n_rows ? row_nnz[r0 + k] : 0;
+    const long long tot = block_sum_1024(s, wsum);
+    if (threadIdx.x == 0) block_sums[blk] = tot;
+}
+__device__ __forceinline__ void row_block_offsets(const int64_t* row_nnz, int64_t n_rows, const int64_t* block_sums,
+                                                  int64_t* indptr, unsigned blk, long long* wsum) {
+    const int t = threadIdx.x, lane = t & 63, wave = t >> 6;
+    const int64_t r0 = (int64_t)blk * kScanBlock + (int64_t)kScanPer * t;
+    long long v[kScanPer], s = 0;
+#pragma unroll
+    for (int k = 0; k < kScanPer; ++k) {
+        v[k] = r0 + k < n_rows ? row_nnz[r0 + k] : 0;
+        s += v[k];
+    }
+    long long before = 0;
+    for (int b = t; b < (int)blk; b += 1024) before += block_sums[b];
+    before = block_sum_1024(before, wsum);
+    long long incl = s;
+#pragma unroll
+    for (int o = 1; o < 64; o <<= 1) {
+        const unsigned lo = (unsigned)__shfl_up((int)(unsigned)incl, o);
+        const unsigned hi = (unsigned)__shfl_up((int)(unsigned)((unsigned long long)incl >> 32), o);
+        if (lane >= o) incl += (long long)(((unsigned long long)hi << 32) | lo);
+    }
+    __syncthreads();
+    if (lane == 63) wsum[wave] = incl;
+    __syncthreads();
+    for (int w = 0; w < wave; ++w) before += wsum[w];
+    long long run = before + incl - s;
+    if (blk == 0 && t == 0) indptr[0] = 0;
+#pragma unroll
+    for (int k = 0; k < kScanPer; ++k) {
+        run += v[k];
+        if (r0 + k < n_rows) indptr[r0 + k + 1] = run;
+    }
+}
 __global__ void __launch_bounds__(1024) k_row_block_sums(const int64_t* __restrict__ row_nnz, int64_t n_rows,
                                                          int64_t* __restrict__ block_sums) {
     __shared__ long long wsum[16];
-    const int64_t r0 = (int64_t)blockIdx.x * kScanBlock + (int64_t)kScanPer * threadIdx.x;
-    long long s = 0;
-#pragma unroll
-    for (int k = 0; k < kScanPer; ++k) s += r0 + k < n_rows ? row_nnz[r0 + k] : 0;
-    const long long tot = block_sum_1024(s, wsum);
-    if (threadIdx.x == 0) block_sums[blockIdx.x] = tot;
+    row_block_sum(row_nnz, n_rows, block_sums, blockIdx.x, wsum);
 }
 __global__ void __launch_bounds__(1024) k_row_offsets(const int64_t* __restrict__ row_nnz, int64_t n_rows,
                                                       const int64_t* __restrict__ block_sums,
                                                       int64_t* __restrict__ indptr) {
     __shared__ long long wsum[16];
-    const int t = threadIdx.x, lane = t & 63, wave = t >> 6;
-    const int64_t r0 = (int64_t)blockIdx.x * kScanBlock + (int64_t)kScanPer * t;
-    long long v[kScanPer], s = 0;
-#pragma unroll
-    for (int k = 0; k < kScanPer; ++k) {
-        v[k] = r0 + k < n_rows ? row_nnz[r0 + k] : 0;
-        s += v[k];
-    }
-    long long before = 0;
-    for (int b = t; b < (int)blockIdx.x; b += 1024) before += block_sums[b];
-    before = block_sum_1024(before, wsum);
-    long long incl = s;
-#pragma unroll
-    for (int o = 1; o < 64; o <<= 1) {
-        const unsigned lo = (unsigned)__shfl_up((int)(unsigned)incl, o);
-        const unsigned hi = (unsigned)__shfl_up((int)(unsigned)((unsigned long long)incl >> 32), o);
-        if (lane >= o) incl += (long long)(((unsigned long long)hi << 32) | lo);
-    }
-    __syncthreads();
-    if (lane == 63) wsum[wave] = incl;
-    __syncthreads();
-    for (int w = 0; w < wave; ++w) before += wsum[w];
-    long long run = before + incl - s;
-    if (blockIdx.x == 0 && t == 0) indptr[0] = 0;
-#pragma unroll
-    for (int k = 0; k < kScanPer; ++k) {
-        run += v[k];
-        if (r0 + k < n_rows) indptr[r0 + k + 1] = run;
-    }
+    row_block_offsets(row_nnz, n_rows, block_sums, indptr, blockIdx.x, wsum);
 }
 
 __global__ void __launch_bounds__(256) k_csr_fill_masked(const float* x, int64_t n_rows, int n_cols, int64_t ld,
diff --git a/infercnvpy_amd/tl/_infercnv.py b/infercnvpy_amd/tl/_infercnv.py
--- a/infercnvpy_amd/tl/_infercnv.py
+++ b/infercnvpy_amd/tl/_infercnv.py
@@ -265,13 +265,16 @@
                     sums = _engine.column_sums(dm, groups, len(counts))
                     cnt = torch.as_tensor(np.asarray(counts, dtype=np.float64)).cuda()
                     rows = list((sums / cnt[:, None]).to(dm.dtype))
+                elif groups is None and not is_csr and n_obs > 0:
+                    rows = [_engine.column_means(dm)]
                 else:
                     rows = []
                     for gi, n_g in enumerate(counts):
                         sel = None if groups is None else np.nonzero(groups == gi)[0]
                         acc = _engine.column_chain(dm, None, sel, int(n_g))
                         rows.append(_engine.chain_mean(acc, int(n_g), is_csr))
-                ref = torch.stack(_repeat_rows(rows, cats))
+                rows = _repeat_rows(rows, cats)
+                ref = rows[0][None, :] if len(rows) == 1 else torch.stack(rows)
             if ref.shape[0] == 1:
                 ref_lo, ref_hi = ref[0].contiguous(), None
             else:
```
